# KiloHertzian/Open-Headstage

Hardware: AMD Instinct MI355X
Metric: Msamples/s stereo 48 kHz (4×512-tap HRIR conv + 10-band EQ); % HBM3E peak (higher is better)
Workload: dtype f32

## Files before the change

include/ohs_hip.h:

```cpp
#ifndef OHS_HIP_H
#define OHS_HIP_H

#include <stddef.h>
#include <stdint.h>

#ifdef __cplusplus
extern "C" {
#endif

#define OHS_BLOCK_SIZE 512
#define OHS_FFT_SIZE   1024
#define OHS_MAX_EQ_BANDS 64

enum {
    OHS_OK = 0,
    OHS_ERR_INVALID_ARG = 1,
    OHS_ERR_NO_DEVICE = 2,
    OHS_ERR_HIP = 3,
    OHS_ERR_OUTSIDE_NYQUIST = 4,
    OHS_ERR_NEGATIVE_Q = 5,
    OHS_ERR_ALLOC = 6,
    OHS_ERR_IO = 7,
    OHS_ERR_PARSE = 8,
    OHS_ERR_RCCL = 9
};

enum { OHS_PATH_LSL = 0, OHS_PATH_LSR = 1, OHS_PATH_RSL = 2, OHS_PATH_RSR = 3 };

enum {
    OHS_FILTER_PEAK = 0, OHS_FILTER_LOWSHELF = 1, OHS_FILTER_HIGHSHELF = 2, OHS_FILTER_LOWPASS = 3,
    OHS_FILTER_HIGHPASS = 4, OHS_FILTER_BANDPASS = 5, OHS_FILTER_NOTCH = 6, OHS_FILTER_ALLPASS = 7
};

int         ohs_version(void);
const char *ohs_status_string(int status);
const char *ohs_last_error(void);
int         ohs_device_count(int *count);
int         ohs_device_pci_bus_id(int device, char *out, size_t capacity);

int         ohs_debug_fft1024(int device, const float *in, float *out, int inverse, size_t batch);

typedef struct ohs_engine ohs_engine;

int  ohs_engine_create(int device, ohs_engine **out);
int  ohs_engine_clone(const ohs_engine *src, ohs_engine **out);
void ohs_engine_destroy(ohs_engine *e);
int  ohs_engine_set_ir(ohs_engine *e, int path, const float *ir, size_t len);
int  ohs_engine_process_block(ohs_engine *e, const float *in_l, const float *in_r,
                              float *out_l, float *out_r, size_t n);
int  ohs_engine_num_partitions(const ohs_engine *e, int path, size_t *out);
int  ohs_engine_set_realtime(ohs_engine *e, int enable);
int  ohs_rt_configure(int max_resident_per_device, uint64_t idle_polls);
int  ohs_engine_latency_samples(const ohs_engine *e, size_t n, size_t *latency);
int  ohs_engine_debug_rt_stamps(const ohs_engine *e, uint64_t out[16]);
int  ohs_engine_silent_frames(const ohs_engine *e, uint64_t *frames);
int  ohs_engine_set_flush_denormals(ohs_engine *e, int mode);

typedef struct ohs_eq ohs_eq;

int  ohs_biquad_coeffs(int filter_type, float fs, float fc, float q, float gain_db, float out[5]);
int  ohs_eq_create(int device, size_t num_bands, float fs, ohs_eq **out);
void ohs_eq_destroy(ohs_eq *eq);
int  ohs_eq_update_band(ohs_eq *eq, size_t band, float fs, int filter_type, float fc, float q,
                        float gain_db, int enabled);
int  ohs_eq_set_band_coeffs(ohs_eq *eq, size_t band, const float coeffs[5], int enabled);
int  ohs_eq_get_band_coeffs(const ohs_eq *eq, size_t band, float coeffs[5], int *enabled);
int  ohs_eq_process_block(ohs_eq *eq, float *left, float *right, size_t n);
int  ohs_eq_set_exact_specials(ohs_eq *eq, int enable);
int  ohs_eq_set_flush_denormals(ohs_eq *eq, int mode);
int  ohs_eq_reset(ohs_eq *eq);
int  ohs_eq_frequency_response(const ohs_eq *eq, float fs, const float *freqs, size_t n, float *out);

typedef struct ohs_biquad ohs_biquad;
int  ohs_biquad_create(int device, float initial_sample_rate, ohs_biquad **out);
int  ohs_biquad_clone(const ohs_biquad *src, ohs_biquad **out);
void ohs_biquad_destroy(ohs_biquad *f);
int  ohs_biquad_reset_state(ohs_biquad *f);
int  ohs_biquad_set_enabled(ohs_biquad *f, int enabled);
int  ohs_biquad_update_coeffs(ohs_biquad *f, int filter_type, float sample_rate, float center_freq, float q, float gain_db);
int  ohs_biquad_set_coeffs(ohs_biquad *f, const float coeffs[5]);
int  ohs_biquad_process(ohs_biquad *f, float *samples, size_t n);

typedef struct ohs_band_setting {
    int   enabled;
    int   filter_type;
    float frequency;
    float q;
    float gain;
} ohs_band_setting;
int  ohs_autoeq_parse_csv(const char *path, ohs_band_setting *out, size_t capacity, size_t *count);
int  ohs_autoeq_parse_csv_text(const char *text, size_t len, ohs_band_setting *out, size_t capacity,
                               size_t *count);

typedef struct ohs_sofa ohs_sofa;
int  ohs_sofa_open(const char *path, ohs_sofa **out);
enum { OHS_SOFA_RESAMPLE = 1, OHS_SOFA_LOUDNESS = 2, OHS_SOFA_INTERPOLATE = 4, OHS_SOFA_MYSOFA_DEFAULTS = 7 };
int  ohs_sofa_open_ex(const char *path, unsigned flags, float target_fs, ohs_sofa **out);
int  ohs_sofa_loudness_factor(const ohs_sofa *s, float *factor);
int  ohs_sofa_neighbors(const ohs_sofa *s, size_t m, int out[6]);
void ohs_sofa_close(ohs_sofa *s);
int  ohs_sofa_info(const ohs_sofa *s, size_t *M, size_t *R, size_t *N, float *fs);
int  ohs_sofa_position(const ohs_sofa *s, size_t m, float az_el_r[3]);
int  ohs_sofa_spherical_to_cartesian(const float az_el_r[3], float xyz[3]);
int  ohs_sofa_cartesian_to_spherical(const float xyz[3], float az_el_r[3]);
int  ohs_sofa_nearest(const ohs_sofa *s, float az_deg, float el_deg, float radius_m, size_t *index);
int  ohs_sofa_get_ir(const ohs_sofa *s, size_t m, size_t receiver, float *out, size_t capacity);
int  ohs_sofa_get_hrtf_irs(const ohs_sofa *s, float az_deg, float el_deg, float radius_m, float *left,
                           float *right, size_t capacity, float *delay_left, float *delay_right);
int  ohs_sofa_resample_ir(const float *in, size_t n, float fs_in, float fs_out, float *out, size_t capacity,
                          size_t *out_len);

int  ohs_sofa_speaker_irs(const ohs_sofa *sofa, float az_l, float el_l, float az_r, float el_r, float radius_m, float fs,
                          float *const out[4], size_t capacity, size_t lens[4]);
int  ohs_engine_set_speakers(ohs_engine *e, const ohs_sofa *sofa, float az_l, float el_l, float az_r, float el_r,
                             float radius_m, float fs, unsigned *changed_mask);

int  ohs_chain_process(ohs_engine *e, ohs_eq *eq, int bypass, int eq_enable, float gain,
                       float *left, float *right, size_t n);

typedef struct ohs_batch ohs_batch;

int  ohs_batch_create(int device, size_t n_streams, size_t num_bands, ohs_batch **out);
void ohs_batch_destroy(ohs_batch *b);
int  ohs_batch_set_ir(ohs_batch *b, int path, const float *ir, size_t len);
int  ohs_batch_set_speakers(ohs_batch *b, const ohs_sofa *sofa, float az_l, float el_l, float az_r, float el_r,
                            float radius_m, float fs, unsigned *changed_mask);
int  ohs_batch_set_eq_band_coeffs(ohs_batch *b, size_t band, const float coeffs[5], int enabled);
int  ohs_batch_update_eq_band(ohs_batch *b, size_t band, float fs, int filter_type, float fc,
                              float q, float gain_db, int enabled);
int  ohs_batch_set_stream_eq_band_coeffs(ohs_batch *b, size_t stream, size_t band, const float coeffs[5], int enabled);
int  ohs_batch_update_stream_eq_band(ohs_batch *b, size_t stream, size_t band, float fs, int filter_type, float fc,
                                     float q, float gain_db, int enabled);
int  ohs_batch_share_eq_table(ohs_batch *b);
int  ohs_batch_set_eq_enabled(ohs_batch *b, int eq_enable);
int  ohs_batch_set_eq_exact_specials(ohs_batch *b, int enable);
int  ohs_batch_set_flush_denormals(ohs_batch *b, int mode);
int  ohs_batch_set_gain(ohs_batch *b, float gain);
int  ohs_batch_set_conv_plan(ohs_batch *b, int plan);
enum ohs_conv_kernel {
    OHS_CONV_KERNEL_NONE = 0,
    OHS_CONV_KERNEL_BLOCK512_P1 = 1,
    OHS_CONV_KERNEL_HOP1536_P1 = 2,
    OHS_CONV_KERNEL_BLOCK512_TP = 3,
    OHS_CONV_KERNEL_BLOCK2048 = 4,
    OHS_CONV_KERNEL_SEQUENTIAL = 5,
    OHS_CONV_KERNEL_BLOCK8192 = 6,
    OHS_CONV_KERNEL_COUNT = 8
};
int  ohs_batch_last_conv_plan(const ohs_batch *b, int *kernel, int *ranges_per_stream);
int  ohs_batch_conv_plan_counts(ohs_batch *b, uint64_t counts[8] , int reset);
int  ohs_batch_reset(ohs_batch *b);
int  ohs_batch_process(ohs_batch *b, const float *d_in, float *d_out, size_t n_blocks,
                       size_t stream_stride, size_t channel_stride, void *hip_stream);
int  ohs_batch_set_schedule_tables(ohs_batch *b, size_t n_tables, const float *coeffs, const uint8_t *enabled);
int  ohs_batch_process_scheduled(ohs_batch *b, const float *d_in, float *d_out, size_t n_blocks, size_t stream_stride,
                                 size_t channel_stride, size_t seg_blocks, const unsigned *table_idx, const float *gain,
                                 void *hip_stream);
int  ohs_batch_process_scheduled_streams(ohs_batch *b, const float *d_in, float *d_out, size_t n_blocks, size_t stream_stride,
                                         size_t channel_stride, size_t seg_blocks, const unsigned *table_idx, size_t idx_stride,
                                         const float *gain, size_t gain_stride, void *hip_stream);
enum {
    OHS_EQ_FORM_NONE = 0,
    OHS_EQ_FORM_ROW_RING = 1,
    OHS_EQ_FORM_WAVE_RING = 2,
    OHS_EQ_FORM_CONVEYOR = 3
};
int  ohs_batch_last_eq_form(const ohs_batch *b, int *form, int *scheduled);
int  ohs_batch_process_deferred(ohs_batch *b, const float *d_in, float *d_out, size_t n_blocks,
                                size_t stream_stride, size_t channel_stride, void *hip_stream);
int  ohs_batch_join(ohs_batch *b, void *hip_stream);
int  ohs_batch_process_host(ohs_batch *b, const float *h_in, float *h_out, size_t n_blocks,
                            size_t stream_stride, size_t channel_stride, size_t chunk_blocks);
int  ohs_batch_sync(ohs_batch *b, void *hip_stream);
int  ohs_batch_set_profiling(ohs_batch *b, int enable);
int  ohs_batch_profile_read(ohs_batch *b, double *eq_ms, double *conv_ms, uint64_t *n_calls,
                            uint64_t *eq_launches, uint64_t *conv_launches);
int  ohs_batch_profile_eq_clock(ohs_batch *b, double *shader_ghz, double *wave_us);
int  ohs_batch_algorithmic_bytes(const ohs_batch *b, size_t n_blocks, uint64_t *bytes);
int  ohs_batch_kernel_bytes(const ohs_batch *b, size_t n_blocks, uint64_t *eq_bytes, uint64_t *conv_bytes);

typedef struct ohs_node_batch ohs_node_batch;
int  ohs_node_batch_create(int n_devices, const int *devices, size_t streams_total, size_t num_bands,
                           ohs_node_batch **out);
void ohs_node_batch_destroy(ohs_node_batch *nb);
int  ohs_node_batch_shard(const ohs_node_batch *nb, int slot, int *device, size_t *first_stream, size_t *n_streams);
int  ohs_node_batch_device_batch(ohs_node_batch *nb, int slot, ohs_batch **out);
int  ohs_node_batch_set_tables(ohs_node_batch *nb, const float *const irs[4], const size_t lens[4],
                               const float *eq_coeffs, const int *eq_enabled);
int  ohs_node_batch_set_ir(ohs_node_batch *nb, int path, const float *ir, size_t len);
int  ohs_node_batch_set_speakers(ohs_node_batch *nb, const ohs_sofa *sofa, float az_l, float el_l, float az_r, float el_r,
                                 float radius_m, float fs, unsigned *changed_mask);
int  ohs_node_batch_set_eq_band_coeffs(ohs_node_batch *nb, size_t band, const float coeffs[5], int enabled);
int  ohs_node_batch_set_stream_eq_band_coeffs(ohs_node_batch *nb, size_t stream, size_t band, const float coeffs[5],
                                              int enabled);
int  ohs_node_batch_share_eq_table(ohs_node_batch *nb);
int  ohs_node_batch_set_eq_enabled(ohs_node_batch *nb, int eq_enable);
int  ohs_node_batch_set_gain(ohs_node_batch *nb, float gain);
int  ohs_node_batch_set_conv_plan(ohs_node_batch *nb, int plan);
int  ohs_node_batch_reset(ohs_node_batch *nb);
int  ohs_node_batch_process_host(ohs_node_batch *nb, const float *h_in, float *h_out, size_t n_blocks,
                                 size_t stream_stride, size_t channel_stride, size_t chunk_blocks);
int  ohs_node_batch_process(ohs_node_batch *nb, const float *const d_in[], float *const d_out[], size_t n_blocks,
                            size_t stream_stride, size_t channel_stride);
int  ohs_node_batch_sync(ohs_node_batch *nb);
int  ohs_node_batch_stream(ohs_node_batch *nb, int slot, void **hip_stream);
int  ohs_node_batch_timer_begin(ohs_node_batch *nb);
int  ohs_node_batch_timer_end(ohs_node_batch *nb, float *ms_per_slot);
int  ohs_node_batch_rccl_info(const ohs_node_batch *nb, int *comm_size, int *rccl_loaded);

#ifdef __cplusplus
}
#endif
#endif
```

open_headstage_amd/_ffi.py:

```python
from __future__ import annotations

import ctypes as C
import os

HERE = os.path.dirname(os.path.abspath(__file__))
EXP_LIB_PATH = os.path.join(HERE, "libohs_hip_exp.so")
_env_lib = os.environ.get("OHS_LIB")
LIB_PATH = EXP_LIB_PATH if _env_lib == "exp" else (_env_lib or os.path.join(HERE, "libohs_hip.so"))

OHS_OK = 0
OHS_ERR_INVALID_ARG = 1
OHS_ERR_NO_DEVICE = 2
OHS_ERR_HIP = 3
OHS_ERR_OUTSIDE_NYQUIST = 4
OHS_ERR_NEGATIVE_Q = 5
OHS_ERR_ALLOC = 6
OHS_ERR_IO = 7
OHS_ERR_PARSE = 8
OHS_ERR_RCCL = 9

class BandSettingC(C.Structure):
    _fields_ = [("enabled", C.c_int), ("filter_type", C.c_int), ("frequency", C.c_float),
                ("q", C.c_float), ("gain", C.c_float)]


fp = C.POINTER(C.c_float)
vp = C.c_void_p
vpp = C.POINTER(C.c_void_p)

PROTOTYPES = {
    "ohs_version": (C.c_int, []),
    "ohs_status_string": (C.c_char_p, [C.c_int]),
    "ohs_last_error": (C.c_char_p, []),
    "ohs_device_count": (C.c_int, [C.POINTER(C.c_int)]),
    "ohs_device_pci_bus_id": (C.c_int, [C.c_int, C.c_char_p, C.c_size_t]),
    "ohs_debug_fft1024": (C.c_int, [C.c_int, fp, fp, C.c_int, C.c_size_t]),
    "ohs_engine_create": (C.c_int, [C.c_int, vpp]),
    "ohs_engine_clone": (C.c_int, [vp, vpp]),
    "ohs_engine_destroy": (None, [vp]),
    "ohs_engine_set_ir": (C.c_int, [vp, C.c_int, fp, C.c_size_t]),
    "ohs_engine_process_block": (C.c_int, [vp, vp, vp, vp, vp, C.c_size_t]),
    "ohs_engine_num_partitions": (C.c_int, [vp, C.c_int, C.POINTER(C.c_size_t)]),
    "ohs_engine_set_realtime": (C.c_int, [vp, C.c_int]),
    "ohs_rt_configure": (C.c_int, [C.c_int, C.c_uint64]),
    "ohs_engine_latency_samples": (C.c_int, [vp, C.c_size_t, C.POINTER(C.c_size_t)]),
    "ohs_engine_silent_frames": (C.c_int, [vp, C.POINTER(C.c_uint64)]),
    "ohs_engine_debug_rt_stamps": (C.c_int, [vp, C.POINTER(C.c_uint64)]),
    "ohs_biquad_coeffs": (C.c_int, [C.c_int, C.c_float, C.c_float, C.c_float, C.c_float, fp]),
    "ohs_biquad_create": (C.c_int, [C.c_int, C.c_float, vpp]),
    "ohs_biquad_clone": (C.c_int, [vp, vpp]),
    "ohs_biquad_destroy": (None, [vp]),
    "ohs_biquad_reset_state": (C.c_int, [vp]),
    "ohs_biquad_set_enabled": (C.c_int, [vp, C.c_int]),
    "ohs_biquad_update_coeffs": (C.c_int, [vp, C.c_int, C.c_float, C.c_float, C.c_float, C.c_float]),
    "ohs_biquad_set_coeffs": (C.c_int, [vp, fp]),
    "ohs_biquad_process": (C.c_int, [vp, vp, C.c_size_t]),
    "ohs_eq_create": (C.c_int, [C.c_int, C.c_size_t, C.c_float, vpp]),
    "ohs_eq_destroy": (None, [vp]),
    "ohs_eq_update_band": (C.c_int, [vp, C.c_size_t, C.c_float, C.c_int, C.c_float, C.c_float,
                                     C.c_float, C.c_int]),
    "ohs_eq_set_band_coeffs": (C.c_int, [vp, C.c_size_t, fp, C.c_int]),
    "ohs_eq_get_band_coeffs": (C.c_int, [vp, C.c_size_t, fp, C.POINTER(C.c_int)]),
    "ohs_eq_process_block": (C.c_int, [vp, vp, vp, C.c_size_t]),
    "ohs_eq_reset": (C.c_int, [vp]),
    "ohs_eq_set_exact_specials": (C.c_int, [vp, C.c_int]),
    "ohs_eq_set_flush_denormals": (C.c_int, [vp, C.c_int]),
    "ohs_engine_set_flush_denormals": (C.c_int, [vp, C.c_int]),
    "ohs_batch_set_flush_denormals": (C.c_int, [vp, C.c_int]),
    "ohs_batch_set_eq_exact_specials": (C.c_int, [vp, C.c_int]),
    "ohs_eq_frequency_response": (C.c_int, [vp, C.c_float, fp, C.c_size_t, fp]),
    "ohs_autoeq_parse_csv": (C.c_int, [C.c_char_p, C.POINTER(BandSettingC), C.c_size_t,
                                       C.POINTER(C.c_size_t)]),
    "ohs_autoeq_parse_csv_text": (C.c_int, [C.c_char_p, C.c_size_t, C.POINTER(BandSettingC), C.c_size_t,
                                            C.POINTER(C.c_size_t)]),
    "ohs_sofa_open": (C.c_int, [C.c_char_p, vpp]),
    "ohs_sofa_open_ex": (C.c_int, [C.c_char_p, C.c_uint, C.c_float, vpp]),
    "ohs_sofa_loudness_factor": (C.c_int, [vp, fp]),
    "ohs_sofa_neighbors": (C.c_int, [vp, C.c_size_t, C.POINTER(C.c_int)]),
    "ohs_sofa_close": (None, [vp]),
    "ohs_sofa_info": (C.c_int, [vp, C.POINTER(C.c_size_t), C.POINTER(C.c_size_t), C.POINTER(C.c_size_t),
                                C.POINTER(C.c_float)]),
    "ohs_sofa_position": (C.c_int, [vp, C.c_size_t, fp]),
    "ohs_sofa_spherical_to_cartesian": (C.c_int, [fp, fp]),
    "ohs_sofa_cartesian_to_spherical": (C.c_int, [fp, fp]),
    "ohs_sofa_nearest": (C.c_int, [vp, C.c_float, C.c_float, C.c_float, C.POINTER(C.c_size_t)]),
    "ohs_sofa_get_ir": (C.c_int, [vp, C.c_size_t, C.c_size_t, fp, C.c_size_t]),
    "ohs_sofa_get_hrtf_irs": (C.c_int, [vp, C.c_float, C.c_float, C.c_float, fp, fp, C.c_size_t, fp, fp]),
    "ohs_sofa_resample_ir": (C.c_int, [fp, C.c_size_t, C.c_float, C.c_float, fp, C.c_size_t,
                                       C.POINTER(C.c_size_t)]),
    "ohs_sofa_speaker_irs": (C.c_int, [vp, C.c_float, C.c_float, C.c_float, C.c_float, C.c_float, C.c_float,
                                       C.POINTER(fp), C.c_size_t, C.POINTER(C.c_size_t)]),
    "ohs_engine_set_speakers": (C.c_int, [vp, vp, C.c_float, C.c_float, C.c_float, C.c_float, C.c_float, C.c_float, C.POINTER(C.c_uint)]),
    "ohs_batch_set_speakers": (C.c_int, [vp, vp, C.c_float, C.c_float, C.c_float, C.c_float, C.c_float, C.c_float, C.POINTER(C.c_uint)]),
    "ohs_node_batch_set_speakers": (C.c_int, [vp, vp, C.c_float, C.c_float, C.c_float, C.c_float, C.c_float, C.c_float, C.POINTER(C.c_uint)]),
    "ohs_chain_process": (C.c_int, [vp, vp, C.c_int, C.c_int, C.c_float, vp, vp, C.c_size_t]),
    "ohs_batch_create": (C.c_int, [C.c_int, C.c_size_t, C.c_size_t, vpp]),
    "ohs_batch_destroy": (None, [vp]),
    "ohs_batch_set_ir": (C.c_int, [vp, C.c_int, fp, C.c_size_t]),
    "ohs_batch_set_eq_band_coeffs": (C.c_int, [vp, C.c_size_t, fp, C.c_int]),
    "ohs_batch_update_eq_band": (C.c_int, [vp, C.c_size_t, C.c_float, C.c_int, C.c_float, C.c_float,
                                           C.c_float, C.c_int]),
    "ohs_batch_set_stream_eq_band_coeffs": (C.c_int, [vp, C.c_size_t, C.c_size_t, fp, C.c_int]),
    "ohs_batch_update_stream_eq_band": (C.c_int, [vp, C.c_size_t, C.c_size_t, C.c_float, C.c_int, C.c_float, C.c_float,
                                                  C.c_float, C.c_int]),
    "ohs_batch_share_eq_table": (C.c_int, [vp]),
    "ohs_node_batch_set_stream_eq_band_coeffs": (C.c_int, [vp, C.c_size_t, C.c_size_t, fp, C.c_int]),
    "ohs_node_batch_share_eq_table": (C.c_int, [vp]),
    "ohs_batch_set_eq_enabled": (C.c_int, [vp, C.c_int]),
    "ohs_batch_set_gain": (C.c_int, [vp, C.c_float]),
    "ohs_batch_set_conv_plan": (C.c_int, [vp, C.c_int]),
    "ohs_batch_last_conv_plan": (C.c_int, [vp, C.POINTER(C.c_int), C.POINTER(C.c_int)]),
    "ohs_batch_conv_plan_counts": (C.c_int, [vp, C.POINTER(C.c_uint64), C.c_int]),
    "ohs_batch_profile_eq_clock": (C.c_int, [vp, C.POINTER(C.c_double), C.POINTER(C.c_double)]),
    "ohs_node_batch_set_conv_plan": (C.c_int, [vp, C.c_int]),
    "ohs_batch_reset": (C.c_int, [vp]),
    "ohs_batch_process": (C.c_int, [vp, vp, vp, C.c_size_t, C.c_size_t, C.c_size_t, vp]),
    "ohs_batch_process_deferred": (C.c_int, [vp, vp, vp, C.c_size_t, C.c_size_t, C.c_size_t, vp]),
    "ohs_batch_set_schedule_tables": (C.c_int, [vp, C.c_size_t, fp, C.POINTER(C.c_uint8)]),
    "ohs_batch_process_scheduled": (C.c_int, [vp, vp, vp, C.c_size_t, C.c_size_t, C.c_size_t, C.c_size_t,
                                              C.POINTER(C.c_uint32), fp, vp]),
    "ohs_batch_process_scheduled_streams": (C.c_int, [vp, vp, vp, C.c_size_t, C.c_size_t, C.c_size_t, C.c_size_t,
                                                    C.POINTER(C.c_uint32), C.c_size_t, fp, C.c_size_t, vp]),
    "ohs_batch_last_eq_form": (C.c_int, [vp, C.POINTER(C.c_int), C.POINTER(C.c_int)]),
    "ohs_batch_join": (C.c_int, [vp, vp]),
    "ohs_batch_sync": (C.c_int, [vp, vp]),
    "ohs_batch_process_host": (C.c_int, [vp, vp, vp, C.c_size_t, C.c_size_t, C.c_size_t, C.c_size_t]),
    "ohs_batch_set_profiling": (C.c_int, [vp, C.c_int]),
    "ohs_batch_profile_read": (C.c_int, [vp, C.POINTER(C.c_double), C.POINTER(C.c_double),
                                         C.POINTER(C.c_uint64), C.POINTER(C.c_uint64),
                                         C.POINTER(C.c_uint64)]),
    "ohs_batch_algorithmic_bytes": (C.c_int, [vp, C.c_size_t, C.POINTER(C.c_uint64)]),
    "ohs_batch_kernel_bytes": (C.c_int, [vp, C.c_size_t, C.POINTER(C.c_uint64), C.POINTER(C.c_uint64)]),
    "ohs_node_batch_create": (C.c_int, [C.c_int, C.POINTER(C.c_int), C.c_size_t, C.c_size_t, vpp]),
    "ohs_node_batch_destroy": (None, [vp]),
    "ohs_node_batch_shard": (C.c_int, [vp, C.c_int, C.POINTER(C.c_int), C.POINTER(C.c_size_t), C.POINTER(C.c_size_t)]),
    "ohs_node_batch_device_batch": (C.c_int, [vp, C.c_int, vpp]),
    "ohs_node_batch_set_tables": (C.c_int, [vp, C.POINTER(fp), C.POINTER(C.c_size_t), fp, C.POINTER(C.c_int)]),
    "ohs_node_batch_set_ir": (C.c_int, [vp, C.c_int, fp, C.c_size_t]),
    "ohs_node_batch_set_eq_band_coeffs": (C.c_int, [vp, C.c_size_t, fp, C.c_int]),
    "ohs_node_batch_set_eq_enabled": (C.c_int, [vp, C.c_int]),
    "ohs_node_batch_set_gain": (C.c_int, [vp, C.c_float]),
    "ohs_node_batch_reset": (C.c_int, [vp]),
    "ohs_node_batch_process_host": (C.c_int, [vp, vp, vp, C.c_size_t, C.c_size_t, C.c_size_t, C.c_size_t]),
    "ohs_node_batch_process": (C.c_int, [vp, C.POINTER(C.c_void_p), C.POINTER(C.c_void_p), C.c_size_t, C.c_size_t,
                                         C.c_size_t]),
    "ohs_node_batch_sync": (C.c_int, [vp]),
    "ohs_node_batch_stream": (C.c_int, [vp, C.c_int, vpp]),
    "ohs_node_batch_timer_begin": (C.c_int, [vp]),
    "ohs_node_batch_timer_end": (C.c_int, [vp, fp]),
    "ohs_node_batch_rccl_info": (C.c_int, [vp, C.POINTER(C.c_int), C.POINTER(C.c_int)]),
}


class OhsError(RuntimeError):
    def __init__(self, status: int, detail: str):
        self.status = status
        super().__init__(f"{lib().ohs_status_string(status).decode()} ({status}): {detail}")


DEBUG_PROTOTYPES = {
    "ohs_debug_set_tuning": (C.c_int, [C.c_char_p, C.c_char_p]),
    "ohs_debug_inject_batch_failure": (C.c_int, [C.c_int]),
}

_lib = None
_exp = None


def _load(path: str, extra=None) -> C.CDLL:
    if not os.path.exists(path):
        raise ImportError(
            f"{path} not found: build it with `python -m open_headstage_amd.build` "
            "(hipcc, gfx950). There is no CPU fallback.")
    try:
        import torch
    except ImportError:
        pass
    L = C.CDLL(path)
    for name, (res, args) in {**PROTOTYPES, **(extra or {})}.items():
        fn = getattr(L, name)
        fn.restype = res
        fn.argtypes = args
    return L


def lib() -> C.CDLL:
    global _lib
    if _lib is None:
        _lib = _load(LIB_PATH)
    return _lib


def experiments_lib() -> C.CDLL:
    global _exp
    if _exp is None:
        _exp = _load(EXP_LIB_PATH, DEBUG_PROTOTYPES)
    return _exp


def set_tuning(key: str, value) -> None:
    L = experiments_lib()
    rc = L.ohs_debug_set_tuning(key.encode(), str(value).encode())
    if rc != OHS_OK:
        raise OhsError(rc, L.ohs_last_error().decode(errors="replace"))


def check(status: int, library=None) -> None:
    if status != OHS_OK:
        raise OhsError(status, (library or lib()).ohs_last_error().decode(errors="replace"))
```

open_headstage_amd/csrc/api_batch.hip:

```cpp
#include "api_internal.h"

using namespace ohs;
using namespace ohs_api;
using ohs_host::rbj;

extern "C" {

int ohs_batch_create(int device, size_t n_streams, size_t num_bands, ohs_batch **out)
{
    if (!out) return fail(OHS_ERR_INVALID_ARG, "out is NULL");
    *out = nullptr;
    if (n_streams == 0 || n_streams > (1u << 20)) return fail(OHS_ERR_INVALID_ARG, "n_streams out of range");
    DeviceCtx *ctx = nullptr;
    int rc = get_ctx(device, &ctx);
    if (rc) return rc;
    HIP_TRY(hipSetDevice(device));
    ohs_batch *b = new (std::nothrow) ohs_batch();
    if (!b) return fail(OHS_ERR_ALLOC, "out of host memory");
    b->device = device; b->ctx = ctx;
    if (hipStreamCreateWithFlags(&b->st, hipStreamNonBlocking) != hipSuccess) {
        delete b;
        return fail(OHS_ERR_HIP, "hipStreamCreate failed");
    }
    {
// ... 164 lines not shown
int ohs_batch_conv_plan_counts(ohs_batch *b, uint64_t counts[OHS_CONV_KERNEL_COUNT], int reset)
{
    if (!b || !counts) return fail(OHS_ERR_INVALID_ARG, "NULL argument");
    for (int k = 0; k < OHS_CONV_KERNEL_COUNT; ++k) counts[k] = b->conv.kernel_calls[k];
    if (reset)
        for (int k = 0; k < OHS_CONV_KERNEL_COUNT; ++k) b->conv.kernel_calls[k] = 0;
    return OHS_OK;
}

int ohs_batch_set_gain(ohs_batch *b, float gain)
{
    if (!b) return fail(OHS_ERR_INVALID_ARG, "batch is NULL");
    b->gain = gain;
    return OHS_OK;
}

int ohs_batch_reset(ohs_batch *b)
{
    if (!b) return fail(OHS_ERR_INVALID_ARG, "batch is NULL");
    HIP_TRY(hipSetDevice(b->device));
    DeviceWideSection dws;
    HIP_TRY(hipDeviceSynchronize());
    ConvState &c = b->conv;
    HIP_TRY(hipMemsetAsync(c.d_hist, 0, c.S * (size_t)c.cap * NF * sizeof(float2), b->st));
    HIP_TRY(hipMemsetAsync(c.d_tails, 0, c.S * 2 * 8 * 64 * sizeof(float2), b->st));
    c.tails_lazy = false;
    c.lb_lazy = false; c.lb_valid = 0;
    c.pt_active = false;
    if (c.d_xhist) {
        HIP_TRY(hipMemsetAsync(c.d_xhist, 0, c.S * 2 * (size_t)(2 * c.xh_len) * sizeof(float), b->st));
        c.xh_valid = c.xh_len;
        c.xh_head = 0;
    }
    c.cnt = 0;
    for (int p = 0; p < 4; ++p) c.since[p] = 0;
    int rc = eq_reset(b->eq, b->st);
    if (rc) return rc;
    HIP_TRY(hipStreamSynchronize(b->st));
    b->failed = false;
    b->fail_msg.clear();
    return OHS_OK;
}

static int batch_process_body(ohs_batch *b, const float *d_in, float *d_out, size_t n_blocks,
                              size_t stream_stride, size_t channel_stride, void *hip_stream, bool deferred,
                              const BatchSchedule *sc);

static int batch_process_impl(ohs_batch *b, const float *d_in, float *d_out, size_t n_blocks,
                              size_t stream_stride, size_t channel_stride, void *hip_stream, bool deferred,
                              const BatchSchedule *sc = nullptr)
{
    if (!b || !d_in || !d_out) return fail(OHS_ERR_INVALID_ARG, "NULL argument");
    if (b->failed)
        return fail(OHS_ERR_HIP, "this batch failed in the middle of an earlier call (" + b->fail_msg +
                                     "): its per-stream state is half-advanced; ohs_batch_reset starts it afresh");
    const size_t spans_before = b->spans.size();
    const int rc = batch_process_body(b, d_in, d_out, n_blocks, stream_stride, channel_stride, hip_stream, deferred, sc);
    if (rc == OHS_OK || rc == OHS_ERR_INVALID_ARG) return rc;
    const std::string why = g_err;
    hipStream_t st = (hipStream_t)hip_stream;
    hipEvent_t ev = nullptr;
    if (hipEventCreate(&ev) == hipSuccess) {
        if (hipEventRecord(ev, b->st2) != hipSuccess || hipStreamWaitEvent(st, ev, 0) != hipSuccess)
            hipStreamSynchronize(b->st2);
        b->ev_inflight.push_back(ev);
    } else {
        hipStreamSynchronize(b->st2);
    }
    b->join_pending = false;
    while (b->spans.size() > spans_before) {
        ohs_batch::Span sp = b->spans.back();
        b->spans.pop_back();
        if (sp.a) hipEventDestroy(sp.a);
        if (sp.b) hipEventDestroy(sp.b);
    }
    b->failed = true;
    b->fail_msg = why;
    return fail(rc, why);
}

static int batch_process_body(ohs_batch *b, const float *d_in, float *d_out, size_t n_blocks,
                              size_t stream_stride, size_t channel_stride, void *hip_stream, bool deferred,
                              const BatchSchedule *sc)
{
    if (n_blocks == 0) return OHS_OK;
    if (n_blocks > (size_t)1 << 24) return fail(OHS_ERR_INVALID_ARG, "n_blocks too large");
    const size_t frames = n_blocks * BS;
    if (channel_stride < frames || (b->conv.S > 1 && stream_stride < 2 * frames && stream_stride < channel_stride + frames))
        return fail(OHS_ERR_INVALID_ARG, "strides smaller than the processed region");
    HIP_TRY(hipSetDevice(b->device));
    hipStream_t st = (hipStream_t)hip_stream;
    auto get_event = [&](hipEvent_t *e) -> int {
        if (!b->ev_pool.empty()) { *e = b->ev_pool.back(); b->ev_pool.pop_back(); return OHS_OK; }
        HIP_TRY(hipEventCreate(e));
        return OHS_OK;
    };
    for (size_t i = 0; i < b->ev_inflight.size();) {
        if (hipEventQuery(b->ev_inflight[i]) == hipSuccess) {
            b->ev_pool.push_back(b->ev_inflight[i]);
            b->ev_inflight[i] = b->ev_inflight.back();
            b->ev_inflight.pop_back();
        } else ++i;
    }
    auto span_begin = [&](hipStream_t s_, int kind) -> int {
        if (!b->profiling) return OHS_OK;
        ohs_batch::Span sp; sp.kind = kind; sp.a = nullptr; sp.b = nullptr;
        int rc = get_event(&sp.a); if (rc) return rc;
        rc = get_event(&sp.b); if (rc) return rc;
        HIP_TRY(hipEventRecord(sp.a, s_));
        b->spans.push_back(sp);
        return OHS_OK;
    };
    auto span_end = [&](hipStream_t s_) -> int {
        if (!b->profiling) return OHS_OK;
        HIP_TRY(hipEventRecord(b->spans.back().b, s_));
        return OHS_OK;
    };
    if (b->profiling) b->prof_calls++;

    const bool sched_tabs = sc != nullptr && sc->tab != nullptr;
    bool eq_active = b->eq_enable && eq_any_enabled(b->eq);
    if (sched_tabs) {
        eq_active = false;
        const size_t rows = sc->tab_stride ? b->conv.S : 1;
        for (size_t r = 0; r < rows && b->eq_enable && !eq_active; ++r)
            for (size_t k = 0; k < sc->n_segs && !eq_active; ++k)
                eq_active = eq_schedule_table_any_enabled(b->eq, sc->tab[r * sc->tab_stride + k]);
    }
    ConvGains cg;
    if (sc && sc->d_gain) { cg.tab = sc->d_gain; cg.seg_blocks = (int)sc->seg_blocks; cg.stream_stride = (int)sc->gain_stride; }

    const long long ss = (long long)stream_stride, cs = (long long)channel_stride;
    int rc;
    const bool will_overlap = eq_active && b->overlap && n_blocks >= 64;
    bool chunk_waits = false;
    if (b->join_pending) {
        chunk_waits = will_overlap && b->pend_out == d_out && b->pend_blocks == n_blocks &&
                      b->pend_ss == stream_stride && b->pend_cs == channel_stride;
        if (!chunk_waits) {
            HIP_TRY(hipStreamWaitEvent(st, b->chunk_done[(size_t)b->chunk_done_n - 1], 0));
            b->join_pending = false;
        }
    }
    if (!eq_active) {
#ifdef OHS_EXPERIMENTS
        if (g_inject_batch_failure.load() > 0 && g_inject_batch_failure.fetch_sub(1) == 1)
            return fail(OHS_ERR_HIP, "injected failure (ohs_debug_inject_batch_failure)");
#endif
        rc = span_begin(st, 1); if (rc) return rc;
        rc = conv_launch(b->conv, b->ctx, d_in, ss, cs, d_out, ss, cs, (int)n_blocks, b->gain, st, true, nullptr, nullptr, &cg);
        if (rc) return rc;
        return span_end(st);
    }
    const std::vector<double> &kCut = tuning().overlap_cuts;
    const int nch = (b->overlap && n_blocks >= 64) ? (int)kCut.size() - 1 : 1;
    struct XcdScope {
        ohs_batch *b;
        XcdScope(ohs_batch *b_, int x) : b(b_)
        {
            if (x > 0 && x < 8) { b->eq.xcd_lo = 0; b->eq.xcd_n = x; b->conv.xcd_lo = x; b->conv.xcd_n = 8 - x; }
        }
        ~XcdScope() { b->eq.xcd_lo = 0; b->eq.xcd_n = 8; b->conv.xcd_lo = 0; b->conv.xcd_n = 8; }
    } xcd_scope(b, nch > 1 ? b->xcd_split : 0);
    bool joined = false;
    for (int i = 0; i < nch; ++i) {
        const size_t blk0 = nch == 1 ? 0 : (size_t)(kCut[i] * (double)n_blocks);
        const size_t blk1 = nch == 1 ? n_blocks : (i == nch - 1 ? n_blocks : (size_t)(kCut[i + 1] * (double)n_blocks));
        const size_t off = blk0 * BS;
        const int nb_i = (int)(blk1 - blk0);
        if (nb_i <= 0) {
            if (nch > 1 && deferred) {
                while (b->chunk_done.size() <= (size_t)i) {
                    hipEvent_t ev;
                    HIP_TRY(hipEventCreateWithFlags(&ev, hipEventDisableTiming));
                    b->chunk_done.push_back(ev);
                }
                HIP_TRY(hipEventRecord(b->chunk_done[(size_t)i], b->st2));
            }
            continue;
        }
        if (chunk_waits) HIP_TRY(hipStreamWaitEvent(st, b->chunk_done[(size_t)i], 0));
#ifdef OHS_EXPERIMENTS
        if (g_inject_batch_failure.load() > 0 && g_inject_batch_failure.fetch_sub(1) == 1)
            return fail(OHS_ERR_HIP, "injected failure (ohs_debug_inject_batch_failure)");
#endif
        hipEvent_t ev_a = nullptr, ev_b = nullptr;
        if (b->profiling) {
            ohs_batch::Span sp; sp.kind = 0; sp.a = nullptr; sp.b = nullptr;
            rc = get_event(&sp.a); if (rc) return rc;
            rc = get_event(&sp.b); if (rc) return rc;
            b->spans.push_back(sp);
            ev_a = sp.a; ev_b = sp.b;
        } else if (nch > 1) {
            rc = get_event(&ev_b); if (rc) return rc;
            b->ev_inflight.push_back(ev_b);
        }
        if (sched_tabs && sc->streams)
            rc = eq_launch_scheduled_streams(b->eq, *sc, blk0, (size_t)nb_i, d_in + off, d_out + off, ss, cs, st, ev_a, ev_b);
        else if (sched_tabs) rc = eq_launch_scheduled(b->eq, *sc, blk0, (size_t)nb_i, d_in + off, d_out + off, ss, cs, st, ev_a, ev_b);
        else rc = eq_launch(b->eq, d_in + off, d_out + off, ss, cs, (long long)nb_i * BS, st, nullptr, ev_a, ev_b);
        if (rc) return rc;
        hipStream_t cst = st;
        const bool tail_on_caller = nch > 1 && !deferred && i == nch - 1;
        if (tail_on_caller) {
            hipEvent_t ev;
            rc = get_event(&ev); if (rc) return rc;
            HIP_TRY(hipEventRecord(ev, b->st2));
            HIP_TRY(hipStreamWaitEvent(st, ev, 0));
            b->ev_inflight.push_back(ev);
            joined = true;
        } else if (nch > 1) {
            HIP_TRY(hipStreamWaitEvent(b->st2, ev_b, 0));
            cst = b->st2;
        }
        {
            hipEvent_t cv_a = nullptr, cv_b = nullptr;
            if (b->profiling) {
                ohs_batch::Span sp; sp.kind = 1; sp.a = nullptr; sp.b = nullptr;
                rc = get_event(&sp.a); if (rc) return rc;
                rc = get_event(&sp.b); if (rc) return rc;
                b->spans.push_back(sp);
                cv_a = sp.a; cv_b = sp.b;
            }
            cg.blk_off = (int)blk0;
            rc = conv_launch(b->conv, b->ctx, d_out + off, ss, cs, d_out + off, ss, cs, nb_i, b->gain, cst, true, cv_a, cv_b, &cg);
            if (rc) return rc;
        }
        if (nch > 1 && deferred) {
            while (b->chunk_done.size() <= (size_t)i) {
                hipEvent_t ev;
                HIP_TRY(hipEventCreateWithFlags(&ev, hipEventDisableTiming));
                b->chunk_done.push_back(ev);
            }
            HIP_TRY(hipEventRecord(b->chunk_done[(size_t)i], b->st2));
        }
    }
    b->join_pending = false;
    if (nch > 1 && deferred) {
        b->join_pending = true;
        b->chunk_done_n = nch;
        b->pend_out = d_out; b->pend_blocks = n_blocks; b->pend_ss = stream_stride; b->pend_cs = channel_stride;
    } else if (nch > 1 && !joined) {
        hipEvent_t ev;
        rc = get_event(&ev); if (rc) return rc;
        HIP_TRY(hipEventRecord(ev, b->st2));
        HIP_TRY(hipStreamWaitEvent(st, ev, 0));
        b->ev_inflight.push_back(ev);
    }
    return OHS_OK;
}

int ohs_batch_process(ohs_batch *b, const float *d_in, float *d_out, size_t n_blocks,
                      size_t stream_stride, size_t channel_stride, void *hip_stream)
{
    return batch_process_impl(b, d_in, d_out, n_blocks, stream_stride, channel_stride, hip_stream, false);
}

int ohs_batch_set_schedule_tables(ohs_batch *b, size_t n_tables, const float *coeffs, const uint8_t *enabled)
{
    if (!b) return fail(OHS_ERR_INVALID_ARG, "batch is NULL");
    if (n_tables > 0 && (!coeffs || !enabled)) return fail(OHS_ERR_INVALID_ARG, "NULL argument");
    if (n_tables > ((size_t)1 << 24)) return fail(OHS_ERR_INVALID_ARG, "n_tables too large");
    HIP_TRY(hipSetDevice(b->device));
    return eq_set_schedule_tables(b->eq, n_tables, coeffs, enabled, b->st);
}

int ohs_batch_last_eq_form(const ohs_batch *b, int *form, int *scheduled)
{
    if (!b || !form || !scheduled) return fail(OHS_ERR_INVALID_ARG, "NULL argument");
    *form = b->eq.last_form;
    *scheduled = b->eq.last_scheduled ? 1 : 0;
    return OHS_OK;
}

int ohs_batch_process_scheduled(ohs_batch *b, const float *d_in, float *d_out, size_t n_blocks, size_t stream_stride,
                                size_t channel_stride, size_t seg_blocks, const unsigned *table_idx, const float *gain,
                                void *hip_stream)
{
    if (!b || !d_in || !d_out) return fail(OHS_ERR_INVALID_ARG, "NULL argument");
    if (seg_blocks == 0) return fail(OHS_ERR_INVALID_ARG, "seg_blocks is 0");
    if (n_blocks > (size_t)1 << 24) return fail(OHS_ERR_INVALID_ARG, "n_blocks too large");
    if (b->eq.per_stream)
        return fail(OHS_ERR_INVALID_ARG, "a scheduled call on a handle with per-stream EQ tables is not supported "
                                         "(ohs_batch_share_eq_table goes back to the one shared table)");
    if (table_idx && b->eq.sched_n == 0)
        return fail(OHS_ERR_INVALID_ARG, "table_idx given, but no tables uploaded (ohs_batch_set_schedule_tables)");
    seg_blocks = std::min(seg_blocks, std::max<size_t>(n_blocks, 1));
    const size_t n_segs = (n_blocks + seg_blocks - 1) / seg_blocks;
    if (table_idx)
        for (size_t k = 0; k < n_segs; ++k)
            if (table_idx[k] >= b->eq.sched_n) return fail(OHS_ERR_INVALID_ARG, "table_idx entry out of range");
    if (b->failed || n_blocks == 0)
        return batch_process_impl(b, d_in, d_out, n_blocks, stream_stride, channel_stride, hip_stream, false);
    {
        const size_t frames = n_blocks * BS;
        if (channel_stride < frames || (b->conv.S > 1 && stream_stride < 2 * frames && stream_stride < channel_stride + frames))
            return fail(OHS_ERR_INVALID_ARG, "strides smaller than the processed region");
    }
    auto adopt_table = [&](unsigned t) {
        for (size_t band = 0; band < b->eq.nb; ++band)
            eq_set_shared_band(b->eq, band, &b->eq.sched_coeffs[((size_t)t * b->eq.nb + band) * 5], b->eq.sched_en[(size_t)t * b->eq.nb + band]);
    };
    bool tabs_vary = false, gains_vary = false;
    for (size_t k = 1; k < n_segs; ++k) {
        tabs_vary = tabs_vary || (table_idx && table_idx[k] != table_idx[0]);
        gains_vary = gains_vary || (gain && std::memcmp(&gain[k], &gain[0], sizeof(float)) != 0);
    }
    if (table_idx && !tabs_vary) { adopt_table(table_idx[0]); table_idx = nullptr; }
    if (gain && !gains_vary) { b->gain = gain[0]; gain = nullptr; }
    if (!table_idx && !gain)
        return batch_process_impl(b, d_in, d_out, n_blocks, stream_stride, channel_stride, hip_stream, false);

    HIP_TRY(hipSetDevice(b->device));
    hipStream_t st = (hipStream_t)hip_stream;
    ohs_batch::SchedSlot &slot = b->sched_slot[b->sched_next];
    b->sched_next = (b->sched_next + 1) % ohs_batch::kSchedSlots;
    if (slot.in_use) HIP_TRY(hipEventSynchronize(slot.done));
    slot.in_use = false;
    if (!slot.done) HIP_TRY(hipEventCreateWithFlags(&slot.done, hipEventDisableTiming));
    if (slot.cap < n_segs) {
        if (slot.h) hipHostFree(slot.h);
        if (slot.d) {
            DeviceWideSection dws;
            hipFree(slot.d);
        }
        slot.h = nullptr; slot.d = nullptr; slot.cap = 0;
        const size_t cap = std::max<size_t>(1024, n_segs + n_segs / 2);
        HIP_TRY(hipHostMalloc(reinterpret_cast<void **>(&slot.h), 2 * cap * sizeof(unsigned), hipHostMallocDefault));
        HIP_TRY(hipMalloc(reinterpret_cast<void **>(&slot.d), 2 * cap * sizeof(unsigned)));
        slot.cap = cap;
    }
    BatchSchedule sc;
    sc.seg_blocks = seg_blocks; sc.n_segs = n_segs; sc.tab = table_idx; sc.gain = gain;
    if (table_idx) {
        std::memcpy(slot.h, table_idx, n_segs * sizeof(unsigned));
        HIP_TRY(hipMemcpyAsync(slot.d, slot.h, n_segs * sizeof(unsigned), hipMemcpyHostToDevice, st));
        sc.d_tab = slot.d;
    }
    if (gain) {
        std::memcpy(slot.h + slot.cap, gain, n_segs * sizeof(float));
        HIP_TRY(hipMemcpyAsync(slot.d + slot.cap, slot.h + slot.cap, n_segs * sizeof(float), hipMemcpyHostToDevice, st));
        sc.d_gain = reinterpret_cast<const float *>(slot.d + slot.cap);
    }
    const int rc = batch_process_impl(b, d_in, d_out, n_blocks, stream_stride, channel_stride, hip_stream, false, &sc);
    if (hipEventRecord(slot.done, st) == hipSuccess) slot.in_use = true;
    else hipStreamSynchronize(st);
    if (rc) return rc;
    if (table_idx) adopt_table(table_idx[n_segs - 1]);
    if (gain) b->gain = gain[n_segs - 1];
    return OHS_OK;
}

int ohs_batch_process_scheduled_streams(ohs_batch *b, const float *d_in, float *d_out, size_t n_blocks, size_t stream_stride,
                                        size_t channel_stride, size_t seg_blocks, const unsigned *table_idx, size_t idx_stride,
                                        const float *gain, size_t gain_stride, void *hip_stream)
{
    if (!b || !d_in || !d_out) return fail(OHS_ERR_INVALID_ARG, "NULL argument");
    if (seg_blocks == 0) return fail(OHS_ERR_INVALID_ARG, "seg_blocks is 0");
    if (n_blocks > (size_t)1 << 24) return fail(OHS_ERR_INVALID_ARG, "n_blocks too large");
    if (table_idx && b->eq.per_stream)
        return fail(OHS_ERR_INVALID_ARG, "table_idx on a handle with static per-stream EQ tables is not supported: the schedule "
                                         "tables take their place (ohs_batch_share_eq_table), or pass table_idx = NULL");
    if (table_idx && b->eq.sched_n == 0)
        return fail(OHS_ERR_INVALID_ARG, "table_idx given, but no tables uploaded (ohs_batch_set_schedule_tables)");
    seg_blocks = std::min(seg_blocks, std::max<size_t>(n_blocks, 1));
    const size_t n_segs = (n_blocks + seg_blocks - 1) / seg_blocks, S = b->conv.S;
    if ((table_idx && idx_stride != 0 && idx_stride < n_segs) || (gain && gain_stride != 0 && gain_stride < n_segs))
        return fail(OHS_ERR_INVALID_ARG, "a row stride is 0 (one row for all streams) or >= the number of segments");
    if (S * n_segs > (size_t)0x7fffffff) return fail(OHS_ERR_INVALID_ARG, "schedule too large");
    if (!table_idx) idx_stride = 0;
    if (!gain) gain_stride = 0;
    BatchSchedule sc;
    sc.seg_blocks = seg_blocks; sc.n_segs = n_segs; sc.streams = true;
    if (table_idx) {
        sc.tab = table_idx; sc.tab_stride = idx_stride;
        if (!eq_schedule_streams_scan(b->eq, sc)) return fail(OHS_ERR_INVALID_ARG, "table_idx entry out of range");
    }
    if (b->failed || n_blocks == 0)
        return batch_process_impl(b, d_in, d_out, n_blocks, stream_stride, channel_stride, hip_stream, false);
    {
        const size_t frames = n_blocks * BS;
        if (channel_stride < frames || (S > 1 && stream_stride < 2 * frames && stream_stride < channel_stride + frames))
            return fail(OHS_ERR_INVALID_ARG, "strides smaller than the processed region");
    }
    auto rows_equal = [&](const void *base, size_t stride) {
        const unsigned *p = static_cast<const unsigned *>(base);
        for (size_t s = 1; s < S; ++s)
            if (std::memcmp(p + s * stride, p, n_segs * sizeof(unsigned)) != 0) return false;
        return true;
    };
    if (idx_stride && rows_equal(table_idx, idx_stride)) idx_stride = 0;
    if (gain_stride && rows_equal(gain, gain_stride)) gain_stride = 0;
    struct Restore {
        ohs_batch *b;
        std::vector<float> coeffs; std::vector<int> en; float gain;
        explicit Restore(ohs_batch *b_) : b(b_), coeffs(b_->eq.coeffs), en(b_->eq.en.begin(), b_->eq.en.end()), gain(b_->gain) {}
        ~Restore()
        {
            b->gain = gain;
            if (!b->eq.per_stream)
                for (size_t band = 0; band < b->eq.nb; ++band) eq_set_shared_band(b->eq, band, &coeffs[5 * band], en[band]);
        }
    } restore(b);
    if (!idx_stride && !gain_stride && !b->eq.per_stream)
        return ohs_batch_process_scheduled(b, d_in, d_out, n_blocks, stream_stride, channel_stride, seg_blocks, table_idx, gain, hip_stream);
    auto adopt_table = [&](unsigned t) {
        for (size_t band = 0; band < b->eq.nb; ++band)
            eq_set_shared_band(b->eq, band, &b->eq.sched_coeffs[((size_t)t * b->eq.nb + band) * 5], b->eq.sched_en[(size_t)t * b->eq.nb + band]);
    };
    if (table_idx && !idx_stride) {
        bool vary = false;
        for (size_t k = 1; k < n_segs; ++k) vary = vary || table_idx[k] != table_idx[0];
        if (!vary) { adopt_table(table_idx[0]); table_idx = nullptr; }
    }
    if (gain && !gain_stride) {
        bool vary = false;
        for (size_t k = 1; k < n_segs; ++k) vary = vary || std::memcmp(&gain[k], &gain[0], sizeof(float)) != 0;
// ... 336 lines not shown
```

open_headstage_amd/csrc/eq_quad_ring_asm.inc:

```
#define EQ_QUAD_RING_K 8
#define EQ_QUAD_RING_LOOP \
    "s_mov_b32 vcc_lo, -1\n" \
    "s_mov_b32 vcc_hi, 0x3333ffff\n" \
    ".p2align 5\n" \
    "1:\n" \
    "v_add_f32_dpp v3, v4, v5 wave_ror:1 row_mask:0xf bank_mask:0xf\n" \
    "v_mul_f32_dpp v4, v2, v8 quad_perm:[0,0,0,3] row_mask:0xf bank_mask:0xf\n" \
    "v_nop_e64\n" \
    "v_mul_f32_dpp v6, v3, v7 quad_perm:[0,0,3,3] row_mask:0xf bank_mask:0xf\n" \
    "v_sub_f32_dpp v5, v3, v6 quad_perm:[0,0,1,2] row_mask:0xf bank_mask:0xf\n" \
    "v_add_f32_dpp v2, v4, v5 wave_ror:1 row_mask:0xf bank_mask:0xf\n" \
    "v_mul_f32_dpp v4, v3, v8 quad_perm:[0,0,0,3] row_mask:0xf bank_mask:0xf\n" \
    "v_nop_e64\n" \
    "v_mul_f32_dpp v6, v2, v7 quad_perm:[0,0,3,3] row_mask:0xf bank_mask:0xf\n" \
    "v_sub_f32_dpp v5, v2, v6 quad_perm:[0,0,1,2] row_mask:0xf bank_mask:0xf\n" \
    "v_add_f32_dpp v3, v4, v5 wave_ror:1 row_mask:0xf bank_mask:0xf\n" \
    "v_mul_f32_dpp v4, v2, v8 quad_perm:[0,0,0,3] row_mask:0xf bank_mask:0xf\n" \
    "v_nop_e64\n" \
    "v_mul_f32_dpp v6, v3, v7 quad_perm:[0,0,3,3] row_mask:0xf bank_mask:0xf\n" \
    "v_sub_f32_dpp v5, v3, v6 quad_perm:[0,0,1,2] row_mask:0xf bank_mask:0xf\n" \
    "v_add_f32_dpp v2, v4, v5 wave_ror:1 row_mask:0xf bank_mask:0xf\n" \
    "v_mul_f32_dpp v4, v3, v8 quad_perm:[0,0,0,3] row_mask:0xf bank_mask:0xf\n" \
    "v_nop_e64\n" \
    "v_mul_f32_dpp v6, v2, v7 quad_perm:[0,0,3,3] row_mask:0xf bank_mask:0xf\n" \
    "v_sub_f32_dpp v5, v2, v6 quad_perm:[0,0,1,2] row_mask:0xf bank_mask:0xf\n" \
    "v_add_f32_dpp v3, v4, v5 wave_ror:1 row_mask:0xf bank_mask:0xf\n" \
    "v_mul_f32_dpp v4, v2, v8 quad_perm:[0,0,0,3] row_mask:0xf bank_mask:0xf\n" \
    "v_nop_e64\n" \
    "v_mul_f32_dpp v6, v3, v7 quad_perm:[0,0,3,3] row_mask:0xf bank_mask:0xf\n" \
    "v_sub_f32_dpp v5, v3, v6 quad_perm:[0,0,1,2] row_mask:0xf bank_mask:0xf\n" \
    "v_add_f32_dpp v2, v4, v5 wave_ror:1 row_mask:0xf bank_mask:0xf\n" \
    "v_mul_f32_dpp v4, v3, v8 quad_perm:[0,0,0,3] row_mask:0xf bank_mask:0xf\n" \
    "v_nop_e64\n" \
    "v_mul_f32_dpp v6, v2, v7 quad_perm:[0,0,3,3] row_mask:0xf bank_mask:0xf\n" \
    "v_sub_f32_dpp v5, v2, v6 quad_perm:[0,0,1,2] row_mask:0xf bank_mask:0xf\n" \
    "v_add_f32_dpp v3, v4, v5 wave_ror:1 row_mask:0xf bank_mask:0xf\n" \
    "v_mul_f32_dpp v4, v2, v8 quad_perm:[0,0,0,3] row_mask:0xf bank_mask:0xf\n" \
    "v_nop_e64\n" \
    "v_mul_f32_dpp v6, v3, v7 quad_perm:[0,0,3,3] row_mask:0xf bank_mask:0xf\n" \
    "v_sub_f32_dpp v5, v3, v6 quad_perm:[0,0,1,2] row_mask:0xf bank_mask:0xf\n" \
    "v_add_f32_dpp v2, v4, v5 wave_ror:1 row_mask:0xf bank_mask:0xf\n" \
    "v_mul_f32_dpp v4, v3, v8 quad_perm:[0,0,0,3] row_mask:0xf bank_mask:0xf\n" \
    "buffer_store_dword v2, v0, %[rout], 0 offen offset:64\n" \
    "v_mul_f32_dpp v6, v2, v7 quad_perm:[0,0,3,3] row_mask:0xf bank_mask:0xf\n" \
    "v_sub_f32_dpp v5, v2, v6 quad_perm:[0,0,1,2] row_mask:0xf bank_mask:0xf\n" \
    "v_add_f32_dpp v3, v4, v5 wave_ror:1 row_mask:0xf bank_mask:0xf\n" \
    "v_mul_f32_dpp v4, v2, v8 quad_perm:[0,0,0,3] row_mask:0xf bank_mask:0xf\n" \
    "v_cndmask_b32_dpp v4, v11, v4, vcc quad_perm:[0,1,0,1] row_mask:0xf bank_mask:0xf\n" \
    "v_mul_f32_dpp v6, v3, v7 quad_perm:[0,0,3,3] row_mask:0xf bank_mask:0xf\n" \
    "v_sub_f32_dpp v5, v3, v6 quad_perm:[0,0,1,2] row_mask:0xf bank_mask:0xf\n" \
    "v_add_f32_dpp v2, v4, v5 wave_ror:1 row_mask:0xf bank_mask:0xf\n" \
    "v_mul_f32_dpp v4, v3, v8 quad_perm:[0,0,0,3] row_mask:0xf bank_mask:0xf\n" \
    "buffer_load_dword v11, v1, %[rin], 0 offen offset:512\n" \
    "v_mul_f32_dpp v6, v2, v7 quad_perm:[0,0,3,3] row_mask:0xf bank_mask:0xf\n" \
    "v_sub_f32_dpp v5, v2, v6 quad_perm:[0,0,1,2] row_mask:0xf bank_mask:0xf\n" \
    "v_add_f32_dpp v3, v4, v5 wave_ror:1 row_mask:0xf bank_mask:0xf\n" \
    "v_mul_f32_dpp v4, v2, v8 quad_perm:[0,0,0,3] row_mask:0xf bank_mask:0xf\n" \
    "v_nop_e64\n" \
    "v_mul_f32_dpp v6, v3, v7 quad_perm:[0,0,3,3] row_mask:0xf bank_mask:0xf\n" \
    "v_sub_f32_dpp v5, v3, v6 quad_perm:[0,0,1,2] row_mask:0xf bank_mask:0xf\n" \
    "v_add_f32_dpp v2, v4, v5 wave_ror:1 row_mask:0xf bank_mask:0xf\n" \
    "v_mul_f32_dpp v4, v3, v8 quad_perm:[0,0,0,3] row_mask:0xf bank_mask:0xf\n" \
    "v_nop_e64\n" \
    "v_mul_f32_dpp v6, v2, v7 quad_perm:[0,0,3,3] row_mask:0xf bank_mask:0xf\n" \
    "v_sub_f32_dpp v5, v2, v6 quad_perm:[0,0,1,2] row_mask:0xf bank_mask:0xf\n" \
    "v_add_f32_dpp v3, v4, v5 wave_ror:1 row_mask:0xf bank_mask:0xf\n" \
    "v_mul_f32_dpp v4, v2, v8 quad_perm:[0,0,0,3] row_mask:0xf bank_mask:0xf\n" \
    "v_nop_e64\n" \
    "v_mul_f32_dpp v6, v3, v7 quad_perm:[0,0,3,3] row_mask:0xf bank_mask:0xf\n" \
    "v_sub_f32_dpp v5, v3, v6 quad_perm:[0,0,1,2] row_mask:0xf bank_mask:0xf\n" \
    "v_add_f32_dpp v2, v4, v5 wave_ror:1 row_mask:0xf bank_mask:0xf\n" \
    "v_mul_f32_dpp v4, v3, v8 quad_perm:[0,0,0,3] row_mask:0xf bank_mask:0xf\n" \
    "s_waitcnt vmcnt(21)\n" \
    "s_nop 0\n" \
    "v_mul_f32_dpp v6, v2, v7 quad_perm:[0,0,3,3] row_mask:0xf bank_mask:0xf\n" \
    "v_sub_f32_dpp v5, v2, v6 quad_perm:[0,0,1,2] row_mask:0xf bank_mask:0xf\n" \
    "v_add_f32_dpp v3, v4, v5 wave_ror:1 row_mask:0xf bank_mask:0xf\n" \
    "v_mul_f32_dpp v4, v2, v8 quad_perm:[0,0,0,3] row_mask:0xf bank_mask:0xf\n" \
    "buffer_store_dword v3, v0, %[rout], 0 offen offset:92\n" \
    "v_mul_f32_dpp v6, v3, v7 quad_perm:[0,0,3,3] row_mask:0xf bank_mask:0xf\n" \
    "v_sub_f32_dpp v5, v3, v6 quad_perm:[0,0,1,2] row_mask:0xf bank_mask:0xf\n" \
    "v_add_f32_dpp v2, v4, v5 wave_ror:1 row_mask:0xf bank_mask:0xf\n" \
    "v_mul_f32_dpp v4, v3, v8 quad_perm:[0,0,0,3] row_mask:0xf bank_mask:0xf\n" \
    "v_cndmask_b32_dpp v4, v12, v4, vcc quad_perm:[0,1,2,3] row_mask:0xf bank_mask:0xf\n" \
    "v_mul_f32_dpp v6, v2, v7 quad_perm:[0,0,3,3] row_mask:0xf bank_mask:0xf\n" \
    "v_sub_f32_dpp v5, v2, v6 quad_perm:[0,0,1,2] row_mask:0xf bank_mask:0xf\n" \
    "v_add_f32_dpp v3, v4, v5 wave_ror:1 row_mask:0xf bank_mask:0xf\n" \
    "v_mul_f32_dpp v4, v2, v8 quad_perm:[0,0,0,3] row_mask:0xf bank_mask:0xf\n" \
    "v_nop_e64\n" \
    "v_mul_f32_dpp v6, v3, v7 quad_perm:[0,0,3,3] row_mask:0xf bank_mask:0xf\n" \
    "v_sub_f32_dpp v5, v3, v6 quad_perm:[0,0,1,2] row_mask:0xf bank_mask:0xf\n" \
    "v_add_f32_dpp v2, v4, v5 wave_ror:1 row_mask:0xf bank_mask:0xf\n" \
    "v_mul_f32_dpp v4, v3, v8 quad_perm:[0,0,0,3] row_mask:0xf bank_mask:0xf\n" \
    "v_nop_e64\n" \
    "v_mul_f32_dpp v6, v2, v7 quad_perm:[0,0,3,3] row_mask:0xf bank_mask:0xf\n" \
    "v_sub_f32_dpp v5, v2, v6 quad_perm:[0,0,1,2] row_mask:0xf bank_mask:0xf\n" \
    "v_add_f32_dpp v3, v4, v5 wave_ror:1 row_mask:0xf bank_mask:0xf\n" \
    "v_mul_f32_dpp v4, v2, v8 quad_perm:[0,0,0,3] row_mask:0xf bank_mask:0xf\n" \
    "v_nop_e64\n" \
    "v_mul_f32_dpp v6, v3, v7 quad_perm:[0,0,3,3] row_mask:0xf bank_mask:0xf\n" \
    "v_sub_f32_dpp v5, v3, v6 quad_perm:[0,0,1,2] row_mask:0xf bank_mask:0xf\n" \
    "v_add_f32_dpp v2, v4, v5 wave_ror:1 row_mask:0xf bank_mask:0xf\n" \
    "v_mul_f32_dpp v4, v3, v8 quad_perm:[0,0,0,3] row_mask:0xf bank_mask:0xf\n" \
    "v_nop_e64\n" \
    "v_mul_f32_dpp v6, v2, v7 quad_perm:[0,0,3,3] row_mask:0xf bank_mask:0xf\n" \
    "v_sub_f32_dpp v5, v2, v6 quad_perm:[0,0,1,2] row_mask:0xf bank_mask:0xf\n" \
    "v_add_f32_dpp v3, v4, v5 wave_ror:1 row_mask:0xf bank_mask:0xf\n" \
    "v_mul_f32_dpp v4, v2, v8 quad_perm:[0,0,0,3] row_mask:0xf bank_mask:0xf\n" \
    "v_nop_e64\n" \
    "v_mul_f32_dpp v6, v3, v7 quad_perm:[0,0,3,3] row_mask:0xf bank_mask:0xf\n" \
    "v_sub_f32_dpp v5, v3, v6 quad_perm:[0,0,1,2] row_mask:0xf bank_mask:0xf\n" \
    "v_add_f32_dpp v2, v4, v5 wave_ror:1 row_mask:0xf bank_mask:0xf\n" \
    "v_mul_f32_dpp v4, v3, v8 quad_perm:[0,0,0,3] row_mask:0xf bank_mask:0xf\n" \
    "v_nop_e64\n" \
    "v_mul_f32_dpp v6, v2, v7 quad_perm:[0,0,3,3] row_mask:0xf bank_mask:0xf\n" \
    "v_sub_f32_dpp v5, v2, v6 quad_perm:[0,0,1,2] row_mask:0xf bank_mask:0xf\n" \
    "v_add_f32_dpp v3, v4, v5 wave_ror:1 row_mask:0xf bank_mask:0xf\n" \
    "v_mul_f32_dpp v4, v2, v8 quad_perm:[0,0,0,3] row_mask:0xf bank_mask:0xf\n" \
    "v_nop_e64\n" \
    "v_mul_f32_dpp v6, v3, v7 quad_perm:[0,0,3,3] row_mask:0xf bank_mask:0xf\n" \
    "v_sub_f32_dpp v5, v3, v6 quad_perm:[0,0,1,2] row_mask:0xf bank_mask:0xf\n" \
    "v_add_f32_dpp v2, v4, v5 wave_ror:1 row_mask:0xf bank_mask:0xf\n" \
    "v_mul_f32_dpp v4, v3, v8 quad_perm:[0,0,0,3] row_mask:0xf bank_mask:0xf\n" \
    "buffer_store_dword v2, v0, %[rout], 0 offen offset:128\n" \
    "v_mul_f32_dpp v6, v2, v7 quad_perm:[0,0,3,3] row_mask:0xf bank_mask:0xf\n" \
    "v_sub_f32_dpp v5, v2, v6 quad_perm:[0,0,1,2] row_mask:0xf bank_mask:0xf\n" \
    "v_add_f32_dpp v3, v4, v5 wave_ror:1 row_mask:0xf bank_mask:0xf\n" \
    "v_mul_f32_dpp v4, v2, v8 quad_perm:[0,0,0,3] row_mask:0xf bank_mask:0xf\n" \
    "v_cndmask_b32_dpp v4, v12, v4, vcc quad_perm:[0,1,0,1] row_mask:0xf bank_mask:0xf\n" \
    "v_mul_f32_dpp v6, v3, v7 quad_perm:[0,0,3,3] row_mask:0xf bank_mask:0xf\n" \
    "v_sub_f32_dpp v5, v3, v6 quad_perm:[0,0,1,2] row_mask:0xf bank_mask:0xf\n" \
    "v_add_f32_dpp v2, v4, v5 wave_ror:1 row_mask:0xf bank_mask:0xf\n" \
    "v_mul_f32_dpp v4, v3, v8 quad_perm:[0,0,0,3] row_mask:0xf bank_mask:0xf\n" \
    "buffer_load_dword v12, v1, %[rin], 0 offen offset:576\n" \
    "v_mul_f32_dpp v6, v2, v7 quad_perm:[0,0,3,3] row_mask:0xf bank_mask:0xf\n" \
    "v_sub_f32_dpp v5, v2, v6 quad_perm:[0,0,1,2] row_mask:0xf bank_mask:0xf\n" \
    "v_add_f32_dpp v3, v4, v5 wave_ror:1 row_mask:0xf bank_mask:0xf\n" \
    "v_mul_f32_dpp v4, v2, v8 quad_perm:[0,0,0,3] row_mask:0xf bank_mask:0xf\n" \
    "v_nop_e64\n" \
    "v_mul_f32_dpp v6, v3, v7 quad_perm:[0,0,3,3] row_mask:0xf bank_mask:0xf\n" \
    "v_sub_f32_dpp v5, v3, v6 quad_perm:[0,0,1,2] row_mask:0xf bank_mask:0xf\n" \
    "v_add_f32_dpp v2, v4, v5 wave_ror:1 row_mask:0xf bank_mask:0xf\n" \
    "v_mul_f32_dpp v4, v3, v8 quad_perm:[0,0,0,3] row_mask:0xf bank_mask:0xf\n" \
    "v_nop_e64\n" \
    "v_mul_f32_dpp v6, v2, v7 quad_perm:[0,0,3,3] row_mask:0xf bank_mask:0xf\n" \
    "v_sub_f32_dpp v5, v2, v6 quad_perm:[0,0,1,2] row_mask:0xf bank_mask:0xf\n" \
    "v_add_f32_dpp v3, v4, v5 wave_ror:1 row_mask:0xf bank_mask:0xf\n" \
    "v_mul_f32_dpp v4, v2, v8 quad_perm:[0,0,0,3] row_mask:0xf bank_mask:0xf\n" \
    "v_nop_e64\n" \
    "v_mul_f32_dpp v6, v3, v7 quad_perm:[0,0,3,3] row_mask:0xf bank_mask:0xf\n" \
    "v_sub_f32_dpp v5, v3, v6 quad_perm:[0,0,1,2] row_mask:0xf bank_mask:0xf\n" \
    "v_add_f32_dpp v2, v4, v5 wave_ror:1 row_mask:0xf bank_mask:0xf\n" \
    "v_mul_f32_dpp v4, v3, v8 quad_perm:[0,0,0,3] row_mask:0xf bank_mask:0xf\n" \
    "s_waitcnt vmcnt(21)\n" \
    "s_nop 0\n" \
    "v_mul_f32_dpp v6, v2, v7 quad_perm:[0,0,3,3] row_mask:0xf bank_mask:0xf\n" \
// ... 345 lines not shown
    "v_add_f32_dpp v3, v4, v5 wave_ror:1 row_mask:0xf bank_mask:0xf\n" \
    "v_mul_f32_dpp v4, v2, v8 quad_perm:[0,0,0,3] row_mask:0xf bank_mask:0xf\n" \
    "v_nop_e64\n" \
    "v_mul_f32_dpp v6, v3, v7 quad_perm:[0,0,3,3] row_mask:0xf bank_mask:0xf\n" \
    "v_sub_f32_dpp v5, v3, v6 quad_perm:[0,0,1,2] row_mask:0xf bank_mask:0xf\n" \
    "v_add_f32_dpp v2, v4, v5 wave_ror:1 row_mask:0xf bank_mask:0xf\n" \
    "v_mul_f32_dpp v4, v3, v8 quad_perm:[0,0,0,3] row_mask:0xf bank_mask:0xf\n" \
    "v_nop_e64\n" \
    "v_mul_f32_dpp v6, v2, v7 quad_perm:[0,0,3,3] row_mask:0xf bank_mask:0xf\n" \
    "v_sub_f32_dpp v5, v2, v6 quad_perm:[0,0,1,2] row_mask:0xf bank_mask:0xf\n" \
    "v_add_f32_dpp v3, v4, v5 wave_ror:1 row_mask:0xf bank_mask:0xf\n" \
    "v_mul_f32_dpp v4, v2, v8 quad_perm:[0,0,0,3] row_mask:0xf bank_mask:0xf\n" \
    "v_nop_e64\n" \
    "v_mul_f32_dpp v6, v3, v7 quad_perm:[0,0,3,3] row_mask:0xf bank_mask:0xf\n" \
    "v_sub_f32_dpp v5, v3, v6 quad_perm:[0,0,1,2] row_mask:0xf bank_mask:0xf\n" \
    "v_add_f32_dpp v2, v4, v5 wave_ror:1 row_mask:0xf bank_mask:0xf\n" \
    "v_mul_f32_dpp v4, v3, v8 quad_perm:[0,0,0,3] row_mask:0xf bank_mask:0xf\n" \
    "v_nop_e64\n" \
    "v_mul_f32_dpp v6, v2, v7 quad_perm:[0,0,3,3] row_mask:0xf bank_mask:0xf\n" \
    "v_sub_f32_dpp v5, v2, v6 quad_perm:[0,0,1,2] row_mask:0xf bank_mask:0xf\n" \
    "v_add_f32_dpp v3, v4, v5 wave_ror:1 row_mask:0xf bank_mask:0xf\n" \
    "v_mul_f32_dpp v4, v2, v8 quad_perm:[0,0,0,3] row_mask:0xf bank_mask:0xf\n" \
    "v_nop_e64\n" \
    "v_mul_f32_dpp v6, v3, v7 quad_perm:[0,0,3,3] row_mask:0xf bank_mask:0xf\n" \
    "v_sub_f32_dpp v5, v3, v6 quad_perm:[0,0,1,2] row_mask:0xf bank_mask:0xf\n" \
    "v_add_f32_dpp v2, v4, v5 wave_ror:1 row_mask:0xf bank_mask:0xf\n" \
    "v_mul_f32_dpp v4, v3, v8 quad_perm:[0,0,0,3] row_mask:0xf bank_mask:0xf\n" \
    "buffer_store_dword v2, v0, %[rout], 0 offen offset:448\n" \
    "v_mul_f32_dpp v6, v2, v7 quad_perm:[0,0,3,3] row_mask:0xf bank_mask:0xf\n" \
    "v_sub_f32_dpp v5, v2, v6 quad_perm:[0,0,1,2] row_mask:0xf bank_mask:0xf\n" \
    "v_add_f32_dpp v3, v4, v5 wave_ror:1 row_mask:0xf bank_mask:0xf\n" \
    "v_mul_f32_dpp v4, v2, v8 quad_perm:[0,0,0,3] row_mask:0xf bank_mask:0xf\n" \
    "v_cndmask_b32_dpp v4, v17, v4, vcc quad_perm:[0,1,0,1] row_mask:0xf bank_mask:0xf\n" \
    "v_mul_f32_dpp v6, v3, v7 quad_perm:[0,0,3,3] row_mask:0xf bank_mask:0xf\n" \
    "v_sub_f32_dpp v5, v3, v6 quad_perm:[0,0,1,2] row_mask:0xf bank_mask:0xf\n" \
    "v_add_f32_dpp v2, v4, v5 wave_ror:1 row_mask:0xf bank_mask:0xf\n" \
    "v_mul_f32_dpp v4, v3, v8 quad_perm:[0,0,0,3] row_mask:0xf bank_mask:0xf\n" \
    "buffer_load_dword v17, v1, %[rin], 0 offen offset:896\n" \
    "v_mul_f32_dpp v6, v2, v7 quad_perm:[0,0,3,3] row_mask:0xf bank_mask:0xf\n" \
    "v_sub_f32_dpp v5, v2, v6 quad_perm:[0,0,1,2] row_mask:0xf bank_mask:0xf\n" \
    "v_add_f32_dpp v3, v4, v5 wave_ror:1 row_mask:0xf bank_mask:0xf\n" \
    "v_mul_f32_dpp v4, v2, v8 quad_perm:[0,0,0,3] row_mask:0xf bank_mask:0xf\n" \
    "v_nop_e64\n" \
    "v_mul_f32_dpp v6, v3, v7 quad_perm:[0,0,3,3] row_mask:0xf bank_mask:0xf\n" \
    "v_sub_f32_dpp v5, v3, v6 quad_perm:[0,0,1,2] row_mask:0xf bank_mask:0xf\n" \
    "v_add_f32_dpp v2, v4, v5 wave_ror:1 row_mask:0xf bank_mask:0xf\n" \
    "v_mul_f32_dpp v4, v3, v8 quad_perm:[0,0,0,3] row_mask:0xf bank_mask:0xf\n" \
    "v_nop_e64\n" \
    "v_mul_f32_dpp v6, v2, v7 quad_perm:[0,0,3,3] row_mask:0xf bank_mask:0xf\n" \
    "v_sub_f32_dpp v5, v2, v6 quad_perm:[0,0,1,2] row_mask:0xf bank_mask:0xf\n" \
    "v_add_f32_dpp v3, v4, v5 wave_ror:1 row_mask:0xf bank_mask:0xf\n" \
    "v_mul_f32_dpp v4, v2, v8 quad_perm:[0,0,0,3] row_mask:0xf bank_mask:0xf\n" \
    "v_nop_e64\n" \
    "v_mul_f32_dpp v6, v3, v7 quad_perm:[0,0,3,3] row_mask:0xf bank_mask:0xf\n" \
    "v_sub_f32_dpp v5, v3, v6 quad_perm:[0,0,1,2] row_mask:0xf bank_mask:0xf\n" \
    "v_add_f32_dpp v2, v4, v5 wave_ror:1 row_mask:0xf bank_mask:0xf\n" \
    "v_mul_f32_dpp v4, v3, v8 quad_perm:[0,0,0,3] row_mask:0xf bank_mask:0xf\n" \
    "s_waitcnt vmcnt(21)\n" \
    "s_nop 0\n" \
    "v_mul_f32_dpp v6, v2, v7 quad_perm:[0,0,3,3] row_mask:0xf bank_mask:0xf\n" \
    "v_sub_f32_dpp v5, v2, v6 quad_perm:[0,0,1,2] row_mask:0xf bank_mask:0xf\n" \
    "v_add_f32_dpp v3, v4, v5 wave_ror:1 row_mask:0xf bank_mask:0xf\n" \
    "v_mul_f32_dpp v4, v2, v8 quad_perm:[0,0,0,3] row_mask:0xf bank_mask:0xf\n" \
    "buffer_store_dword v3, v0, %[rout], 0 offen offset:476\n" \
    "v_mul_f32_dpp v6, v3, v7 quad_perm:[0,0,3,3] row_mask:0xf bank_mask:0xf\n" \
    "v_sub_f32_dpp v5, v3, v6 quad_perm:[0,0,1,2] row_mask:0xf bank_mask:0xf\n" \
    "v_add_f32_dpp v2, v4, v5 wave_ror:1 row_mask:0xf bank_mask:0xf\n" \
    "v_mul_f32_dpp v4, v3, v8 quad_perm:[0,0,0,3] row_mask:0xf bank_mask:0xf\n" \
    "v_cndmask_b32_dpp v4, v18, v4, vcc quad_perm:[0,1,2,3] row_mask:0xf bank_mask:0xf\n" \
    "v_mul_f32_dpp v6, v2, v7 quad_perm:[0,0,3,3] row_mask:0xf bank_mask:0xf\n" \
    "v_sub_f32_dpp v5, v2, v6 quad_perm:[0,0,1,2] row_mask:0xf bank_mask:0xf\n" \
    "v_add_f32_dpp v3, v4, v5 wave_ror:1 row_mask:0xf bank_mask:0xf\n" \
    "v_mul_f32_dpp v4, v2, v8 quad_perm:[0,0,0,3] row_mask:0xf bank_mask:0xf\n" \
    "v_nop_e64\n" \
    "v_mul_f32_dpp v6, v3, v7 quad_perm:[0,0,3,3] row_mask:0xf bank_mask:0xf\n" \
    "v_sub_f32_dpp v5, v3, v6 quad_perm:[0,0,1,2] row_mask:0xf bank_mask:0xf\n" \
    "v_add_f32_dpp v2, v4, v5 wave_ror:1 row_mask:0xf bank_mask:0xf\n" \
    "v_mul_f32_dpp v4, v3, v8 quad_perm:[0,0,0,3] row_mask:0xf bank_mask:0xf\n" \
    "v_nop_e64\n" \
    "v_mul_f32_dpp v6, v2, v7 quad_perm:[0,0,3,3] row_mask:0xf bank_mask:0xf\n" \
    "v_sub_f32_dpp v5, v2, v6 quad_perm:[0,0,1,2] row_mask:0xf bank_mask:0xf\n" \
    "v_add_f32_dpp v3, v4, v5 wave_ror:1 row_mask:0xf bank_mask:0xf\n" \
    "v_mul_f32_dpp v4, v2, v8 quad_perm:[0,0,0,3] row_mask:0xf bank_mask:0xf\n" \
    "v_nop_e64\n" \
    "v_mul_f32_dpp v6, v3, v7 quad_perm:[0,0,3,3] row_mask:0xf bank_mask:0xf\n" \
    "v_sub_f32_dpp v5, v3, v6 quad_perm:[0,0,1,2] row_mask:0xf bank_mask:0xf\n" \
    "v_add_f32_dpp v2, v4, v5 wave_ror:1 row_mask:0xf bank_mask:0xf\n" \
    "v_mul_f32_dpp v4, v3, v8 quad_perm:[0,0,0,3] row_mask:0xf bank_mask:0xf\n" \
    "v_nop_e64\n" \
    "v_mul_f32_dpp v6, v2, v7 quad_perm:[0,0,3,3] row_mask:0xf bank_mask:0xf\n" \
    "v_sub_f32_dpp v5, v2, v6 quad_perm:[0,0,1,2] row_mask:0xf bank_mask:0xf\n" \
    "v_add_f32_dpp v3, v4, v5 wave_ror:1 row_mask:0xf bank_mask:0xf\n" \
    "v_mul_f32_dpp v4, v2, v8 quad_perm:[0,0,0,3] row_mask:0xf bank_mask:0xf\n" \
    "v_nop_e64\n" \
    "v_mul_f32_dpp v6, v3, v7 quad_perm:[0,0,3,3] row_mask:0xf bank_mask:0xf\n" \
    "v_sub_f32_dpp v5, v3, v6 quad_perm:[0,0,1,2] row_mask:0xf bank_mask:0xf\n" \
    "v_add_f32_dpp v2, v4, v5 wave_ror:1 row_mask:0xf bank_mask:0xf\n" \
    "v_mul_f32_dpp v4, v3, v8 quad_perm:[0,0,0,3] row_mask:0xf bank_mask:0xf\n" \
    "v_nop_e64\n" \
    "v_mul_f32_dpp v6, v2, v7 quad_perm:[0,0,3,3] row_mask:0xf bank_mask:0xf\n" \
    "v_sub_f32_dpp v5, v2, v6 quad_perm:[0,0,1,2] row_mask:0xf bank_mask:0xf\n" \
    "v_add_f32_dpp v3, v4, v5 wave_ror:1 row_mask:0xf bank_mask:0xf\n" \
    "v_mul_f32_dpp v4, v2, v8 quad_perm:[0,0,0,3] row_mask:0xf bank_mask:0xf\n" \
    "v_nop_e64\n" \
    "v_mul_f32_dpp v6, v3, v7 quad_perm:[0,0,3,3] row_mask:0xf bank_mask:0xf\n" \
    "v_sub_f32_dpp v5, v3, v6 quad_perm:[0,0,1,2] row_mask:0xf bank_mask:0xf\n" \
    "v_add_f32_dpp v2, v4, v5 wave_ror:1 row_mask:0xf bank_mask:0xf\n" \
    "v_mul_f32_dpp v4, v3, v8 quad_perm:[0,0,0,3] row_mask:0xf bank_mask:0xf\n" \
    "buffer_store_dword v2, v0, %[rout], 0 offen offset:512\n" \
    "v_mul_f32_dpp v6, v2, v7 quad_perm:[0,0,3,3] row_mask:0xf bank_mask:0xf\n" \
    "v_sub_f32_dpp v5, v2, v6 quad_perm:[0,0,1,2] row_mask:0xf bank_mask:0xf\n" \
    "v_add_f32_dpp v3, v4, v5 wave_ror:1 row_mask:0xf bank_mask:0xf\n" \
    "v_mul_f32_dpp v4, v2, v8 quad_perm:[0,0,0,3] row_mask:0xf bank_mask:0xf\n" \
    "v_cndmask_b32_dpp v4, v18, v4, vcc quad_perm:[0,1,0,1] row_mask:0xf bank_mask:0xf\n" \
    "v_mul_f32_dpp v6, v3, v7 quad_perm:[0,0,3,3] row_mask:0xf bank_mask:0xf\n" \
    "v_sub_f32_dpp v5, v3, v6 quad_perm:[0,0,1,2] row_mask:0xf bank_mask:0xf\n" \
    "v_add_f32_dpp v2, v4, v5 wave_ror:1 row_mask:0xf bank_mask:0xf\n" \
    "v_mul_f32_dpp v4, v3, v8 quad_perm:[0,0,0,3] row_mask:0xf bank_mask:0xf\n" \
    "buffer_load_dword v18, v1, %[rin], 0 offen offset:960\n" \
    "v_mul_f32_dpp v6, v2, v7 quad_perm:[0,0,3,3] row_mask:0xf bank_mask:0xf\n" \
    "v_sub_f32_dpp v5, v2, v6 quad_perm:[0,0,1,2] row_mask:0xf bank_mask:0xf\n" \
    "v_add_f32_dpp v3, v4, v5 wave_ror:1 row_mask:0xf bank_mask:0xf\n" \
    "v_mul_f32_dpp v4, v2, v8 quad_perm:[0,0,0,3] row_mask:0xf bank_mask:0xf\n" \
    "v_add_u32_e64 v1, v1, v9\n" \
    "v_mul_f32_dpp v6, v3, v7 quad_perm:[0,0,3,3] row_mask:0xf bank_mask:0xf\n" \
    "v_sub_f32_dpp v5, v3, v6 quad_perm:[0,0,1,2] row_mask:0xf bank_mask:0xf\n" \
    "v_add_f32_dpp v2, v4, v5 wave_ror:1 row_mask:0xf bank_mask:0xf\n" \
    "v_mul_f32_dpp v4, v3, v8 quad_perm:[0,0,0,3] row_mask:0xf bank_mask:0xf\n" \
    "v_add_u32_e64 v0, v0, v10\n" \
    "v_mul_f32_dpp v6, v2, v7 quad_perm:[0,0,3,3] row_mask:0xf bank_mask:0xf\n" \
    "v_sub_f32_dpp v5, v2, v6 quad_perm:[0,0,1,2] row_mask:0xf bank_mask:0xf\n" \
    "v_add_f32_dpp v3, v4, v5 wave_ror:1 row_mask:0xf bank_mask:0xf\n" \
    "v_mul_f32_dpp v4, v2, v8 quad_perm:[0,0,0,3] row_mask:0xf bank_mask:0xf\n" \
    "v_nop_e64\n" \
    "v_mul_f32_dpp v6, v3, v7 quad_perm:[0,0,3,3] row_mask:0xf bank_mask:0xf\n" \
    "v_sub_f32_dpp v5, v3, v6 quad_perm:[0,0,1,2] row_mask:0xf bank_mask:0xf\n" \
    "v_add_f32_dpp v2, v4, v5 wave_ror:1 row_mask:0xf bank_mask:0xf\n" \
    "v_mul_f32_dpp v4, v3, v8 quad_perm:[0,0,0,3] row_mask:0xf bank_mask:0xf\n" \
    "s_waitcnt vmcnt(21)\n" \
    "s_add_u32 %[cnt], %[cnt], 1\n" \
    "v_mul_f32_dpp v6, v2, v7 quad_perm:[0,0,3,3] row_mask:0xf bank_mask:0xf\n" \
    "v_sub_f32_dpp v5, v2, v6 quad_perm:[0,0,1,2] row_mask:0xf bank_mask:0xf\n" \
    "v_add_f32_dpp v3, v4, v5 wave_ror:1 row_mask:0xf bank_mask:0xf\n" \
    "v_mul_f32_dpp v4, v2, v8 quad_perm:[0,0,0,3] row_mask:0xf bank_mask:0xf\n" \
    "buffer_store_dword v3, v0, %[rout], 0 offen offset:28\n" \
    "v_mul_f32_dpp v6, v3, v7 quad_perm:[0,0,3,3] row_mask:0xf bank_mask:0xf\n" \
    "v_sub_f32_dpp v5, v3, v6 quad_perm:[0,0,1,2] row_mask:0xf bank_mask:0xf\n" \
    "v_add_f32_dpp v2, v4, v5 wave_ror:1 row_mask:0xf bank_mask:0xf\n" \
    "v_mul_f32_dpp v4, v3, v8 quad_perm:[0,0,0,3] row_mask:0xf bank_mask:0xf\n" \
    "v_cndmask_b32_dpp v4, v11, v4, vcc quad_perm:[0,1,2,3] row_mask:0xf bank_mask:0xf\n" \
    "v_mul_f32_dpp v6, v2, v7 quad_perm:[0,0,3,3] row_mask:0xf bank_mask:0xf\n" \
    "v_sub_f32_dpp v5, v2, v6 quad_perm:[0,0,1,2] row_mask:0xf bank_mask:0xf\n" \
    "s_cbranch_scc0 1b\n" \
    "s_waitcnt vmcnt(0)\n" \
    "s_nop 1\n"
```

open_headstage_amd/csrc/eq_quad_ring_body.hpp:

```cpp
#pragma once
#include "kernels.h"
#include "eq_ring64_body.hpp"
#include "eq_quad_ring_asm.inc"

namespace ohs {

constexpr int kQuadGroup = 16;
constexpr int kQuadK = EQ_QUAD_RING_K;
constexpr int kQp0003 = 0xC0, kQp0033 = 0xF0, kQp0012 = 0x90, kQp0101 = 0x44;

struct QuadRegs { float Z0, Z1, Zp, G, P; };

__device__ __forceinline__ void eq_quad_ring_wave(const float *in, float *out, long long stream_stride, long long ch_stride,
                                                  long long n, int n_chains, int nb, const EqPassTable &tab,
                                                  float *__restrict__ state, long long chain)
{
    constexpr int G = kQuadGroup, K = kQuadK;
    static_assert(K == 8, "the operand list below names x0 .. x7");
    if (chain >= n_chains) return;
    const int lane = threadIdx.x & 63, q = lane >> 2, role = lane & 3;
    const int n32 = (int)n;
    const bool band = q < nb, conv = q >= 12;
    const int j = band ? q : 0;
    const float C1 = role < 2 ? 1.0f : !band ? 0.0f : role == 2 ? tab.a2[j] : tab.a1[j];
    const float C2 = !band ? (role < 2 ? 0.0f : 1.0f) : role == 0 ? tab.b2[j] : role == 1 ? tab.b1[j] : role == 2 ? tab.b0[j] : 1.0f;
    const long long base = (chain >> 1) * stream_stride + (chain & 1) * ch_stride;
    const float *src0 = in + base;
    float *dst0 = out + base;
    float *state0 = state + chain * (kEqStateSlots * 2);
    const bool st_band = band && role >= 2;
    const unsigned state_off = (unsigned)(tab.slot[j] * 2 + (role == 2 ? 1 : 0)) * 4u;
    const float s_init = st_band ? ring2_ld(state0, state_off) : 0.0f;
    float s_save = s_init;
    const int t_in = 4 * q + 2;
    const int xs = (role == 0 ? 71 : role == 1 ? 69 : role == 2 ? 62 : 60) - 4 * q;
    const int ss = (role == 0 ? -1 : -3) - 4 * q;
    const bool st_lane = conv && (role == 0 || role == 3), inj_lane = conv && role >= 2;
    auto load_x = [&](int g) -> float {
        const int i = g * G + xs;
        return (conv && (unsigned)i < (unsigned)n32) ? ring2_ld(src0, (unsigned)i * 4u) : 0.0f;
    };
    QuadRegs r = {0.0f, 0.0f, 0.0f, 0.0f, 0.0f};
    float xcur = load_x(-1), xnext = load_x(0);

    const int g_hi = (n32 + 1) / G;
    const int iters = g_hi - 5 >= K ? (g_hi - 5) / K : 0;
    const int g1 = iters ? g_hi : -1, g0 = iters ? g_hi - iters * K : -1;
    float x2 = 0.0f, x3 = 0.0f, x4 = 0.0f, x5 = 0.0f, x6 = 0.0f, x7 = 0.0f;
    if (iters) {
        x2 = load_x(g0 + 2); x3 = load_x(g0 + 3); x4 = load_x(g0 + 4);
        x5 = load_x(g0 + 5); x6 = load_x(g0 + 6); x7 = load_x(g0 + 7);
    }

    auto group_cpp = [&](int g) {
        const float xnext2 = load_x(g + 2);
        auto step = [&](float &zc, const float zo, int s) {
            const int stp = g * G + s;
            zc = dpp_mov<kWaveRor1>(r.Zp, r.Zp) + r.G;
            r.Zp = dpp_mov<kQp0003>(zo, zo) * C2;
            if (s == 8 || s == 15) {
                const int yi = stp + ss;
                if (st_lane && (unsigned)yi < (unsigned)n32) ring2_st(dst0, (unsigned)yi * 4u, zc);
            } else if (s == 9) {
                const float xb = dpp_mov<kQp0101>(xcur, xcur);
                r.Zp = inj_lane ? xb : r.Zp;
            } else if (s == 16) {
                r.Zp = inj_lane ? xnext : r.Zp;
            }
            r.P = dpp_mov<kQp0033>(zc, zc) * C1;
            r.G = dpp_mov<kQp0012>(zc, zc) - r.P;
            if (st_band && stp == t_in) r.G = s_init;
            if (st_band && stp == n32 + t_in) s_save = r.G;
        };
#pragma unroll 1
        for (int s = 1; s <= G; s += 2) {
            step(r.Z1, r.Z0, s);
            step(r.Z0, r.Z1, s + 1);
        }
        xcur = xnext;
        xnext = xnext2;
    };

    const int g_total = (n32 + 62 + G - 1) / G;
    int g = -1;
    const int head_end = iters ? g0 : g_total;
#pragma unroll 1
    for (; g < head_end; ++g) group_cpp(g);
    if (iters) {
        const unsigned bytes = (unsigned)n32 * 4u;
        const ring64_rsrc_t rin = ring64_rsrc(src0, bytes), rout = ring64_rsrc(dst0, bytes);
        unsigned voff_st = st_lane ? (unsigned)(G * (g0 - 1) + 8 + ss) * 4u : 0xFFFFF000u;
        unsigned voff_ld = conv ? (unsigned)(G * g0 + xs) * 4u : 0xFFFFF000u;
        const unsigned inc_ld = conv ? 4u * G * K : 0u, inc_st = st_lane ? 4u * G * K : 0u;
        unsigned cnt = 0u - (unsigned)__builtin_amdgcn_readfirstlane(iters);
        asm volatile(
            "s_nop 4\n"
            EQ_QUAD_RING_LOOP
            : [Z0] "+{v2}"(r.Z0), [Z1] "+{v3}"(r.Z1), [Zp] "+{v4}"(r.Zp), [Gr] "+{v5}"(r.G), [P] "+{v6}"(r.P),
              [vs] "+{v0}"(voff_st), [vl] "+{v1}"(voff_ld), [x0] "+{v11}"(xcur), [x1] "+{v12}"(xnext), [x2] "+{v13}"(x2),
              [x3] "+{v14}"(x3), [x4] "+{v15}"(x4), [x5] "+{v16}"(x5), [x6] "+{v17}"(x6), [x7] "+{v18}"(x7), [cnt] "+s"(cnt)
            : [C1] "{v7}"(C1), [C2] "{v8}"(C2), [incl] "{v9}"(inc_ld), [incs] "{v10}"(inc_st), [rin] "s"(rin), [rout] "s"(rout)
            : "memory", "scc", "vcc");
        g = g1;
#pragma unroll 1
        for (; g < g_total; ++g) group_cpp(g);
    }
    if (st_band) ring2_st(state0, state_off, s_save);
}

}
```

open_headstage_amd/csrc/tuning.cpp:

```cpp
#include "tuning.h"

#include <algorithm>
#include <cstdio>
#include <cstdlib>
#include <mutex>

namespace ohs {

namespace {
Tuning g_tuning;

#ifdef OHS_EXPERIMENTS
bool parse_ints(const std::string &v, int *out, int n)
{
    const char *p = v.c_str();
    for (int i = 0; i < n; ++i) {
        char *end = nullptr;
        const long x = strtol(p, &end, 10);
        if (end == p) return false;
        out[i] = (int)x;
        p = (*end == ',') ? end + 1 : end;
    }
    return true;
}

const struct { const char *env, *key; } kEnvKeys[] = {
    {"OHS_P1_TARGET_WAVES", "p1_target_waves"}, {"OHS_P1_ROUNDS", "p1_rounds"}, {"OHS_P1_OWN_TAILS", "p1_own_tails"},
    {"OHS_P1_STAGGER", "p1_stagger"}, {"OHS_P1_PRIO", "p1_prio"}, {"OHS_P1_WEIGHTS", "p1_weights"},
    {"OHS_P1_LAZY_STATE", "p1_lazy_state"}, {"OHS_P1_XCD", "p1_xcd"}, {"OHS_EQ_XCD", "eq_xcd"},
    {"OHS_EQ_CONVEYOR", "eq_conveyor"}, {"OHS_EQ_RING_V1", "eq_ring_v1"}, {"OHS_EQ_NO_PRIO", "eq_no_prio"}, {"OHS_EQ_FORM", "eq_form"},
    {"OHS_EQ_WG_WAVES", "eq_wg_waves"}, {"OHS_EQ_LDS", "eq_lds"}, {"OHS_NO_OVERLAP", "no_overlap"},
    {"OHS_FORCE_OVERLAP", "force_overlap"}, {"OHS_XCD_SPLIT", "xcd_split"}, {"OHS_OVERLAP_CUTS", "overlap_cuts"},
    {"OHS_CONV_CU_MASK", "conv_cu_mask"}, {"OHS_MAC_NO_XCD", "mac_no_xcd"}, {"OHS_HOST_PIPE_TRACE", "host_pipe_trace"},
    {"OHS_HOST_PIPE_FLAT_PRIORITIES", "host_pipe_flat_priorities"}, {"OHS_RT_MAX_RESIDENT", "rt_max_resident"},
    {"OHS_RT_IDLE_POLLS", "rt_idle_polls"}, {"OHS_RT_POLL_SLEEP", "rt_poll_sleep"},
    {"OHS_NODE_SHARED_DEVICE", "node_shared_device_rehearsal"},
};
std::once_flag g_env_once;
void load_env()
{
    for (const auto &e : kEnvKeys)
        if (const char *v = getenv(e.env))
            if (!tuning_set(e.key, v)) fprintf(stderr, "[ohs experiments] %s=%s ignored\n", e.env, v);
}
#endif
}

const Tuning &tuning()
{
#ifdef OHS_EXPERIMENTS
    std::call_once(g_env_once, load_env);
#endif
    return g_tuning;
}

Tuning &tuning_rt()
{
#ifdef OHS_EXPERIMENTS
    std::call_once(g_env_once, load_env);
#endif
    return g_tuning;
}

#ifdef OHS_EXPERIMENTS
bool tuning_set(const std::string &key, const std::string &value)
{
    Tuning &t = g_tuning;
    int v[4] = {0, 0, 0, 0};
    auto one = [&](int *dst) { if (!parse_ints(value, v, 1)) return false; *dst = v[0]; return true; };
    if (key == "p1_target_waves") { t.p1_target_waves = atoll(value.c_str()); return true; }
    if (key == "p1_rounds") return one(&t.p1_rounds) && (t.p1_rounds = (t.p1_rounds >= 1 && t.p1_rounds <= 4) ? t.p1_rounds : 1);
    if (key == "p1_own_tails") return one(&t.p1_own_tails);
    if (key == "p1_stagger") return one(&t.p1_stagger);
    if (key == "p1_prio") return one(&t.p1_prio);
    if (key == "p1_lazy_state") return one(&t.p1_lazy_state);
    if (key == "p1_weights") {
        if (!parse_ints(value, v, 4)) return false;
        for (int i = 0; i < 4; ++i) if (v[i] <= 0 || v[i] >= 100000) return false;
        for (int i = 0; i < 4; ++i) t.p1_weights[i] = v[i];
        return true;
    }
    if (key == "p1_xcd" || key == "eq_xcd") {
        int *lo = key == "p1_xcd" ? &t.p1_xcd_lo : &t.eq_xcd_lo, *n = key == "p1_xcd" ? &t.p1_xcd_n : &t.eq_xcd_n;
        if (value.empty() || value == "off") { *lo = 0; *n = 0; return true; }
        if (!parse_ints(value, v, 2) || v[1] < 1 || v[0] < 0 || v[0] + v[1] > 8) return false;
        *lo = v[0]; *n = v[1];
        return true;
    }
    if (key == "eq_conveyor") return one(&t.eq_conveyor);
    if (key == "eq_ring_v1") return one(&t.eq_ring_v1);
    if (key == "eq_no_prio") return one(&t.eq_no_prio);
    if (key == "eq_form") return one(&t.eq_form);
    if (key == "eq_wg_waves") {
        if (!one(&t.eq_wg_waves)) return false;
        const int w = t.eq_wg_waves;
        if (!(w == 0 || w == 1 || w == 2 || w == 4 || w == 8 || w == 16)) { t.eq_wg_waves = 0; return false; }
        return true;
    }
    if (key == "eq_lds") { if (!one(&t.eq_lds)) return false; if (t.eq_lds < 0 || t.eq_lds > 65536) t.eq_lds = 0; return true; }
    if (key == "no_overlap") return one(&t.no_overlap);
    if (key == "force_overlap") return one(&t.force_overlap);
    if (key == "xcd_split") { if (!one(&t.xcd_split)) return false; if (t.xcd_split < 0 || t.xcd_split > 7) t.xcd_split = 0; return true; }
    if (key == "overlap_cuts") {
        std::vector<double> c = {0.0};
        const char *p = value.c_str();
        while (*p && c.size() < 16) {
            char *end = nullptr;
            const double x = strtod(p, &end);
            if (end == p) break;
            if (x > c.back() && x < 1.0) c.push_back(x);
            p = (*end == ',') ? end + 1 : end;
        }
        c.push_back(1.0);
        if (c.size() < 3) return false;
        t.overlap_cuts = c;
        return true;
    }
    if (key == "conv_cu_mask") {
        std::vector<unsigned> m;
        const char *p = value.c_str();
        while (*p) {
            char *end = nullptr;
            const unsigned long x = strtoul(p, &end, 16);
            if (end == p) break;
            m.push_back((unsigned)x);
            p = (*end == ',') ? end + 1 : end;
        }
        t.conv_cu_mask = m;
        return true;
    }
    if (key == "mac_no_xcd") return one(&t.mac_no_xcd);
    if (key == "lb_skip") return one(&t.lb_skip);
    if (key == "xb_min_p") return one(&t.xb_min_p);
    if (key == "xb_min_blocks") return one(&t.xb_min_blocks);
    if (key == "xb_min_streams_p2") return one(&t.xb_min_streams_p2);
    if (key == "xb_stagger") { if (!one(&t.xb_stagger)) return false; t.xb_stagger = std::max(0, std::min(t.xb_stagger, 64)); return true; }
    if (key == "xb_run") return one(&t.xb_run);
    if (key == "xb_skip") return one(&t.xb_skip);
    if (key == "lb_seg_windows") { if (!one(&t.lb_seg_windows)) return false; if (t.lb_seg_windows < 64) t.lb_seg_windows = 64; return true; }
    if (key == "lb_min_p") { if (!one(&t.lb_min_p)) return false; if (t.lb_min_p < 2) t.lb_min_p = 2; return true; }
    if (key == "host_pipe_trace") return one(&t.host_pipe_trace);
    if (key == "host_pipe_flat_priorities") return one(&t.host_pipe_flat_priorities);
    if (key == "node_shared_device_rehearsal") return one(&t.node_shared_device_rehearsal);
    if (key == "node_inject_table_failure_slot") return one(&t.node_inject_table_failure_slot);
    if (key == "rt_max_resident") { int v = 0; if (!one(&v)) return false; rt_max_resident_store(v); return true; }
    if (key == "rt_idle_polls") { rt_idle_polls_store(strtoull(value.c_str(), nullptr, 10)); return true; }
    if (key == "rt_poll_sleep") { if (!one(v)) return false; t.rt_poll_sleep = (unsigned)v[0]; return true; }
    return false;
}
#endif

}
```

open_headstage_amd/csrc/tuning.h:

```cpp
#pragma once
#include "experiments.h"

#include <string>
#include <vector>

namespace ohs {

struct Tuning {
    long long p1_target_waves = 0;
    int p1_rounds = 1;
    int p1_own_tails = 1;
    int p1_stagger = 0;
    int p1_prio = 0;
    int p1_weights[4] = {1425, 1128, 825, 622};
    int p1_lazy_state = 1;
    int p1_xcd_lo = 0, p1_xcd_n = 0;
    int eq_xcd_lo = 0, eq_xcd_n = 0;
    int eq_conveyor = 0;
    int eq_ring_v1 = 0;
    int eq_no_prio = 0;
    int eq_form = 0;
    int eq_wg_waves = 0;
    int eq_lds = 0;
    int no_overlap = 0, force_overlap = 0;
    int xcd_split = 0;
    std::vector<double> overlap_cuts = {0.0, 0.25, 0.5, 0.75, 0.92, 0.98, 1.0};
    std::vector<unsigned> conv_cu_mask;
    int mac_no_xcd = 0;
    int lb_min_p = 2;
    int lb_seg_windows = 131072;
    int xb_min_p = 2;
    int xb_min_blocks = 128;
    int xb_min_streams_p2 = 32;
    int xb_stagger = 1;
    int xb_skip = 0;
    int xb_run = 0;
    int lb_skip = 0;
    int host_pipe_trace = 0, host_pipe_flat_priorities = 0;
    int node_shared_device_rehearsal = 0;
    int node_inject_table_failure_slot = 0;
    int rt_max_resident = -1;
    unsigned long long rt_idle_polls = 3000000ull;
    unsigned rt_poll_sleep = 0;
};

const Tuning &tuning();
Tuning &tuning_rt();
inline int rt_max_resident_load() { return __atomic_load_n(&tuning().rt_max_resident, __ATOMIC_RELAXED); }
inline unsigned long long rt_idle_polls_load() { return __atomic_load_n(&tuning().rt_idle_polls, __ATOMIC_RELAXED); }
inline void rt_max_resident_store(int v) { __atomic_store_n(&tuning_rt().rt_max_resident, v, __ATOMIC_RELAXED); }
inline void rt_idle_polls_store(unsigned long long v) { __atomic_store_n(&tuning_rt().rt_idle_polls, v, __ATOMIC_RELAXED); }
#ifdef OHS_EXPERIMENTS
bool tuning_set(const std::string &key, const std::string &value);
#endif

}
```

Baseline: 26130.

## Geometric overlap chunk plan for wave-ring EQ and asm remainder tail

Replaces the fixed fractional overlap cut table with a planner that, when the EQ pass uses the wave-ring form, sizes chunks geometrically from a small tail chunk, with a minimum block floor. The aim is to shorten the final non-overlapped EQ/convolution stage and pipeline the two stages better. The hand-written DPP ring assembly also gains a remainder path, so leftover groups that are not a multiple of the unroll factor stay in asm instead of falling back to the C++ loop. A test-only plan query API is exported. Costs are more code complexity, the risk of chunk sizes that suit some block counts poorly, and correctness risk in the register rotation of the asm tail.

After: 26130 (median of 2 runs). About the same (+0.0%).

```diff
diff --git a/include/ohs_hip.h b/include/ohs_hip.h
--- a/include/ohs_hip.h
+++ b/include/ohs_hip.h
@@ -166,6 +166,7 @@
     OHS_EQ_FORM_CONVEYOR = 3
 };
 int  ohs_batch_last_eq_form(const ohs_batch *b, int *form, int *scheduled);
+int  ohs_batch_overlap_plan(size_t n_blocks, int wave_ring, size_t *cuts, size_t cap, size_t *n_chunks);
 int  ohs_batch_process_deferred(ohs_batch *b, const float *d_in, float *d_out, size_t n_blocks,
                                 size_t stream_stride, size_t channel_stride, void *hip_stream);
 int  ohs_batch_join(ohs_batch *b, void *hip_stream);
diff --git a/open_headstage_amd/_ffi.py b/open_headstage_amd/_ffi.py
--- a/open_headstage_amd/_ffi.py
+++ b/open_headstage_amd/_ffi.py
@@ -122,6 +122,7 @@
     "ohs_batch_process_scheduled_streams": (C.c_int, [vp, vp, vp, C.c_size_t, C.c_size_t, C.c_size_t, C.c_size_t,
                                                     C.POINTER(C.c_uint32), C.c_size_t, fp, C.c_size_t, vp]),
     "ohs_batch_last_eq_form": (C.c_int, [vp, C.POINTER(C.c_int), C.POINTER(C.c_int)]),
+    "ohs_batch_overlap_plan": (C.c_int, [C.c_size_t, C.c_int, C.POINTER(C.c_size_t), C.c_size_t, C.POINTER(C.c_size_t)]),
     "ohs_batch_join": (C.c_int, [vp, vp]),
     "ohs_batch_sync": (C.c_int, [vp, vp]),
     "ohs_batch_process_host": (C.c_int, [vp, vp, vp, C.c_size_t, C.c_size_t, C.c_size_t, C.c_size_t]),
diff --git a/open_headstage_amd/csrc/api_batch.hip b/open_headstage_amd/csrc/api_batch.hip
--- a/open_headstage_amd/csrc/api_batch.hip
+++ b/open_headstage_amd/csrc/api_batch.hip
@@ -340,8 +340,10 @@
         if (rc) return rc;
         return span_end(st);
     }
-    const std::vector<double> &kCut = tuning().overlap_cuts;
-    const int nch = (b->overlap && n_blocks >= 64) ? (int)kCut.size() - 1 : 1;
+    const OverlapPlan plan = (b->overlap && n_blocks >= 64)
+        ? overlap_plan(n_blocks, eq_pass_takes_wave_ring(ss, cs, (long long)frames, (int)b->eq.chains, 1, b->eq.exact_specials), tuning())
+        : OverlapPlan();
+    const int nch = plan.n;
     struct XcdScope {
         ohs_batch *b;
         XcdScope(ohs_batch *b_, int x) : b(b_)
@@ -352,8 +354,8 @@
     } xcd_scope(b, nch > 1 ? b->xcd_split : 0);
     bool joined = false;
     for (int i = 0; i < nch; ++i) {
-        const size_t blk0 = nch == 1 ? 0 : (size_t)(kCut[i] * (double)n_blocks);
-        const size_t blk1 = nch == 1 ? n_blocks : (i == nch - 1 ? n_blocks : (size_t)(kCut[i + 1] * (double)n_blocks));
+        const size_t blk0 = nch == 1 ? 0 : plan.cut[i];
+        const size_t blk1 = nch == 1 ? n_blocks : plan.cut[i + 1];
         const size_t off = blk0 * BS;
         const int nb_i = (int)(blk1 - blk0);
         if (nb_i <= 0) {
@@ -451,6 +453,17 @@
     if (n_tables > ((size_t)1 << 24)) return fail(OHS_ERR_INVALID_ARG, "n_tables too large");
     HIP_TRY(hipSetDevice(b->device));
     return eq_set_schedule_tables(b->eq, n_tables, coeffs, enabled, b->st);
+}
+
+int ohs_batch_overlap_plan(size_t n_blocks, int wave_ring, size_t *cuts, size_t cap, size_t *n_chunks)
+{
+    if (!cuts || !n_chunks) return fail(OHS_ERR_INVALID_ARG, "NULL argument");
+    const OverlapPlan plan = n_blocks >= 64 ? overlap_plan(n_blocks, wave_ring != 0, tuning()) : OverlapPlan();
+    if (cap < (size_t)plan.n + 1) return fail(OHS_ERR_INVALID_ARG, "cuts holds fewer than n_chunks + 1 entries");
+    for (int i = 0; i < plan.n; ++i) cuts[i] = plan.cut[i];
+    cuts[plan.n] = n_blocks;
+    *n_chunks = (size_t)plan.n;
+    return OHS_OK;
 }
 
 int ohs_batch_last_eq_form(const ohs_batch *b, int *form, int *scheduled)
diff --git a/open_headstage_amd/csrc/eq_quad_ring_asm.inc b/open_headstage_amd/csrc/eq_quad_ring_asm.inc
--- a/open_headstage_amd/csrc/eq_quad_ring_asm.inc
+++ b/open_headstage_amd/csrc/eq_quad_ring_asm.inc
@@ -1,7 +1,9 @@
 #define EQ_QUAD_RING_K 8
-#define EQ_QUAD_RING_LOOP \
+#define EQ_QUAD_RING_RUN \
     "s_mov_b32 vcc_lo, -1\n" \
     "s_mov_b32 vcc_hi, 0x3333ffff\n" \
+    "s_cmp_eq_u32 %[cnt], 0\n" \
+    "s_cbranch_scc1 3f\n" \
     ".p2align 5\n" \
     "1:\n" \
     "v_add_f32_dpp v3, v4, v5 wave_ror:1 row_mask:0xf bank_mask:0xf\n" \
@@ -653,5 +655,588 @@
     "v_mul_f32_dpp v6, v2, v7 quad_perm:[0,0,3,3] row_mask:0xf bank_mask:0xf\n" \
     "v_sub_f32_dpp v5, v2, v6 quad_perm:[0,0,1,2] row_mask:0xf bank_mask:0xf\n" \
     "s_cbranch_scc0 1b\n" \
+    "3:\n" \
+    "s_cmp_eq_u32 %[rem], 0\n" \
+    "s_cbranch_scc1 2f\n" \
+    "v_add_f32_dpp v3, v4, v5 wave_ror:1 row_mask:0xf bank_mask:0xf\n" \
+    "v_mul_f32_dpp v4, v2, v8 quad_perm:[0,0,0,3] row_mask:0xf bank_mask:0xf\n" \
+    "v_nop_e64\n" \
+    "v_mul_f32_dpp v6, v3, v7 quad_perm:[0,0,3,3] row_mask:0xf bank_mask:0xf\n" \
+    "v_sub_f32_dpp v5, v3, v6 quad_perm:[0,0,1,2] row_mask:0xf bank_mask:0xf\n" \
+    "v_add_f32_dpp v2, v4, v5 wave_ror:1 row_mask:0xf bank_mask:0xf\n" \
+    "v_mul_f32_dpp v4, v3, v8 quad_perm:[0,0,0,3] row_mask:0xf bank_mask:0xf\n" \
+    "v_nop_e64\n" \
+    "v_mul_f32_dpp v6, v2, v7 quad_perm:[0,0,3,3] row_mask:0xf bank_mask:0xf\n" \
+    "v_sub_f32_dpp v5, v2, v6 quad_perm:[0,0,1,2] row_mask:0xf bank_mask:0xf\n" \
+    "v_add_f32_dpp v3, v4, v5 wave_ror:1 row_mask:0xf bank_mask:0xf\n" \
+    "v_mul_f32_dpp v4, v2, v8 quad_perm:[0,0,0,3] row_mask:0xf bank_mask:0xf\n" \
+    "v_nop_e64\n" \
+    "v_mul_f32_dpp v6, v3, v7 quad_perm:[0,0,3,3] row_mask:0xf bank_mask:0xf\n" \
+    "v_sub_f32_dpp v5, v3, v6 quad_perm:[0,0,1,2] row_mask:0xf bank_mask:0xf\n" \
+    "v_add_f32_dpp v2, v4, v5 wave_ror:1 row_mask:0xf bank_mask:0xf\n" \
+    "v_mul_f32_dpp v4, v3, v8 quad_perm:[0,0,0,3] row_mask:0xf bank_mask:0xf\n" \
+    "v_nop_e64\n" \
+    "v_mul_f32_dpp v6, v2, v7 quad_perm:[0,0,3,3] row_mask:0xf bank_mask:0xf\n" \
+    "v_sub_f32_dpp v5, v2, v6 quad_perm:[0,0,1,2] row_mask:0xf bank_mask:0xf\n" \
+    "v_add_f32_dpp v3, v4, v5 wave_ror:1 row_mask:0xf bank_mask:0xf\n" \
+    "v_mul_f32_dpp v4, v2, v8 quad_perm:[0,0,0,3] row_mask:0xf bank_mask:0xf\n" \
+    "v_nop_e64\n" \
+    "v_mul_f32_dpp v6, v3, v7 quad_perm:[0,0,3,3] row_mask:0xf bank_mask:0xf\n" \
+    "v_sub_f32_dpp v5, v3, v6 quad_perm:[0,0,1,2] row_mask:0xf bank_mask:0xf\n" \
+    "v_add_f32_dpp v2, v4, v5 wave_ror:1 row_mask:0xf bank_mask:0xf\n" \
+    "v_mul_f32_dpp v4, v3, v8 quad_perm:[0,0,0,3] row_mask:0xf bank_mask:0xf\n" \
+    "v_nop_e64\n" \
+    "v_mul_f32_dpp v6, v2, v7 quad_perm:[0,0,3,3] row_mask:0xf bank_mask:0xf\n" \
+    "v_sub_f32_dpp v5, v2, v6 quad_perm:[0,0,1,2] row_mask:0xf bank_mask:0xf\n" \
+    "v_add_f32_dpp v3, v4, v5 wave_ror:1 row_mask:0xf bank_mask:0xf\n" \
+    "v_mul_f32_dpp v4, v2, v8 quad_perm:[0,0,0,3] row_mask:0xf bank_mask:0xf\n" \
+    "v_nop_e64\n" \
+    "v_mul_f32_dpp v6, v3, v7 quad_perm:[0,0,3,3] row_mask:0xf bank_mask:0xf\n" \
+    "v_sub_f32_dpp v5, v3, v6 quad_perm:[0,0,1,2] row_mask:0xf bank_mask:0xf\n" \
+    "v_add_f32_dpp v2, v4, v5 wave_ror:1 row_mask:0xf bank_mask:0xf\n" \
+    "v_mul_f32_dpp v4, v3, v8 quad_perm:[0,0,0,3] row_mask:0xf bank_mask:0xf\n" \
+    "buffer_store_dword v2, v0, %[rout], 0 offen offset:64\n" \
+    "v_mul_f32_dpp v6, v2, v7 quad_perm:[0,0,3,3] row_mask:0xf bank_mask:0xf\n" \
+    "v_sub_f32_dpp v5, v2, v6 quad_perm:[0,0,1,2] row_mask:0xf bank_mask:0xf\n" \
+    "v_add_f32_dpp v3, v4, v5 wave_ror:1 row_mask:0xf bank_mask:0xf\n" \
+    "v_mul_f32_dpp v4, v2, v8 quad_perm:[0,0,0,3] row_mask:0xf bank_mask:0xf\n" \
+    "v_cndmask_b32_dpp v4, v11, v4, vcc quad_perm:[0,1,0,1] row_mask:0xf bank_mask:0xf\n" \
+    "v_mul_f32_dpp v6, v3, v7 quad_perm:[0,0,3,3] row_mask:0xf bank_mask:0xf\n" \
+    "v_sub_f32_dpp v5, v3, v6 quad_perm:[0,0,1,2] row_mask:0xf bank_mask:0xf\n" \
+    "v_add_f32_dpp v2, v4, v5 wave_ror:1 row_mask:0xf bank_mask:0xf\n" \
+    "v_mul_f32_dpp v4, v3, v8 quad_perm:[0,0,0,3] row_mask:0xf bank_mask:0xf\n" \
+    "buffer_load_dword v11, v1, %[rin], 0 offen offset:512\n" \
+    "v_mul_f32_dpp v6, v2, v7 quad_perm:[0,0,3,3] row_mask:0xf bank_mask:0xf\n" \
+    "v_sub_f32_dpp v5, v2, v6 quad_perm:[0,0,1,2] row_mask:0xf bank_mask:0xf\n" \
+    "v_add_f32_dpp v3, v4, v5 wave_ror:1 row_mask:0xf bank_mask:0xf\n" \
+    "v_mul_f32_dpp v4, v2, v8 quad_perm:[0,0,0,3] row_mask:0xf bank_mask:0xf\n" \
+    "v_nop_e64\n" \
+    "v_mul_f32_dpp v6, v3, v7 quad_perm:[0,0,3,3] row_mask:0xf bank_mask:0xf\n" \
+    "v_sub_f32_dpp v5, v3, v6 quad_perm:[0,0,1,2] row_mask:0xf bank_mask:0xf\n" \
+    "v_add_f32_dpp v2, v4, v5 wave_ror:1 row_mask:0xf bank_mask:0xf\n" \
+    "v_mul_f32_dpp v4, v3, v8 quad_perm:[0,0,0,3] row_mask:0xf bank_mask:0xf\n" \
+    "v_nop_e64\n" \
+    "v_mul_f32_dpp v6, v2, v7 quad_perm:[0,0,3,3] row_mask:0xf bank_mask:0xf\n" \
+    "v_sub_f32_dpp v5, v2, v6 quad_perm:[0,0,1,2] row_mask:0xf bank_mask:0xf\n" \
+    "v_add_f32_dpp v3, v4, v5 wave_ror:1 row_mask:0xf bank_mask:0xf\n" \
+    "v_mul_f32_dpp v4, v2, v8 quad_perm:[0,0,0,3] row_mask:0xf bank_mask:0xf\n" \
+    "v_nop_e64\n" \
+    "v_mul_f32_dpp v6, v3, v7 quad_perm:[0,0,3,3] row_mask:0xf bank_mask:0xf\n" \
+    "v_sub_f32_dpp v5, v3, v6 quad_perm:[0,0,1,2] row_mask:0xf bank_mask:0xf\n" \
+    "v_add_f32_dpp v2, v4, v5 wave_ror:1 row_mask:0xf bank_mask:0xf\n" \
+    "v_mul_f32_dpp v4, v3, v8 quad_perm:[0,0,0,3] row_mask:0xf bank_mask:0xf\n" \
+    "s_waitcnt vmcnt(21)\n" \
+    "s_cmp_eq_u32 %[rem], 1\n" \
+    "v_mul_f32_dpp v6, v2, v7 quad_perm:[0,0,3,3] row_mask:0xf bank_mask:0xf\n" \
+    "v_sub_f32_dpp v5, v2, v6 quad_perm:[0,0,1,2] row_mask:0xf bank_mask:0xf\n" \
+    "v_add_f32_dpp v3, v4, v5 wave_ror:1 row_mask:0xf bank_mask:0xf\n" \
+    "v_mul_f32_dpp v4, v2, v8 quad_perm:[0,0,0,3] row_mask:0xf bank_mask:0xf\n" \
+    "buffer_store_dword v3, v0, %[rout], 0 offen offset:92\n" \
+    "v_mul_f32_dpp v6, v3, v7 quad_perm:[0,0,3,3] row_mask:0xf bank_mask:0xf\n" \
+    "v_sub_f32_dpp v5, v3, v6 quad_perm:[0,0,1,2] row_mask:0xf bank_mask:0xf\n" \
+    "v_add_f32_dpp v2, v4, v5 wave_ror:1 row_mask:0xf bank_mask:0xf\n" \
+    "v_mul_f32_dpp v4, v3, v8 quad_perm:[0,0,0,3] row_mask:0xf bank_mask:0xf\n" \
+    "v_cndmask_b32_dpp v4, v12, v4, vcc quad_perm:[0,1,2,3] row_mask:0xf bank_mask:0xf\n" \
+    "v_mul_f32_dpp v6, v2, v7 quad_perm:[0,0,3,3] row_mask:0xf bank_mask:0xf\n" \
+    "v_sub_f32_dpp v5, v2, v6 quad_perm:[0,0,1,2] row_mask:0xf bank_mask:0xf\n" \
+    "s_cbranch_scc1 2f\n" \
+    "s_nop 0\n" \
+    "v_add_f32_dpp v3, v4, v5 wave_ror:1 row_mask:0xf bank_mask:0xf\n" \
+    "v_mul_f32_dpp v4, v2, v8 quad_perm:[0,0,0,3] row_mask:0xf bank_mask:0xf\n" \
+    "v_nop_e64\n" \
+    "v_mul_f32_dpp v6, v3, v7 quad_perm:[0,0,3,3] row_mask:0xf bank_mask:0xf\n" \
+    "v_sub_f32_dpp v5, v3, v6 quad_perm:[0,0,1,2] row_mask:0xf bank_mask:0xf\n" \
+    "v_add_f32_dpp v2, v4, v5 wave_ror:1 row_mask:0xf bank_mask:0xf\n" \
+    "v_mul_f32_dpp v4, v3, v8 quad_perm:[0,0,0,3] row_mask:0xf bank_mask:0xf\n" \
+    "v_nop_e64\n" \
+    "v_mul_f32_dpp v6, v2, v7 quad_perm:[0,0,3,3] row_mask:0xf bank_mask:0xf\n" \
+    "v_sub_f32_dpp v5, v2, v6 quad_perm:[0,0,1,2] row_mask:0xf bank_mask:0xf\n" \
+    "v_add_f32_dpp v3, v4, v5 wave_ror:1 row_mask:0xf bank_mask:0xf\n" \
+    "v_mul_f32_dpp v4, v2, v8 quad_perm:[0,0,0,3] row_mask:0xf bank_mask:0xf\n" \
+    "v_nop_e64\n" \
+    "v_mul_f32_dpp v6, v3, v7 quad_perm:[0,0,3,3] row_mask:0xf bank_mask:0xf\n" \
+    "v_sub_f32_dpp v5, v3, v6 quad_perm:[0,0,1,2] row_mask:0xf bank_mask:0xf\n" \
+    "v_add_f32_dpp v2, v4, v5 wave_ror:1 row_mask:0xf bank_mask:0xf\n" \
+    "v_mul_f32_dpp v4, v3, v8 quad_perm:[0,0,0,3] row_mask:0xf bank_mask:0xf\n" \
+    "v_nop_e64\n" \
+    "v_mul_f32_dpp v6, v2, v7 quad_perm:[0,0,3,3] row_mask:0xf bank_mask:0xf\n" \
+    "v_sub_f32_dpp v5, v2, v6 quad_perm:[0,0,1,2] row_mask:0xf bank_mask:0xf\n" \
+    "v_add_f32_dpp v3, v4, v5 wave_ror:1 row_mask:0xf bank_mask:0xf\n" \
+    "v_mul_f32_dpp v4, v2, v8 quad_perm:[0,0,0,3] row_mask:0xf bank_mask:0xf\n" \
+    "v_nop_e64\n" \
+    "v_mul_f32_dpp v6, v3, v7 quad_perm:[0,0,3,3] row_mask:0xf bank_mask:0xf\n" \
+    "v_sub_f32_dpp v5, v3, v6 quad_perm:[0,0,1,2] row_mask:0xf bank_mask:0xf\n" \
+    "v_add_f32_dpp v2, v4, v5 wave_ror:1 row_mask:0xf bank_mask:0xf\n" \
+    "v_mul_f32_dpp v4, v3, v8 quad_perm:[0,0,0,3] row_mask:0xf bank_mask:0xf\n" \
+    "v_nop_e64\n" \
+    "v_mul_f32_dpp v6, v2, v7 quad_perm:[0,0,3,3] row_mask:0xf bank_mask:0xf\n" \
+    "v_sub_f32_dpp v5, v2, v6 quad_perm:[0,0,1,2] row_mask:0xf bank_mask:0xf\n" \
+    "v_add_f32_dpp v3, v4, v5 wave_ror:1 row_mask:0xf bank_mask:0xf\n" \
+    "v_mul_f32_dpp v4, v2, v8 quad_perm:[0,0,0,3] row_mask:0xf bank_mask:0xf\n" \
+    "v_nop_e64\n" \
+    "v_mul_f32_dpp v6, v3, v7 quad_perm:[0,0,3,3] row_mask:0xf bank_mask:0xf\n" \
+    "v_sub_f32_dpp v5, v3, v6 quad_perm:[0,0,1,2] row_mask:0xf bank_mask:0xf\n" \
+    "v_add_f32_dpp v2, v4, v5 wave_ror:1 row_mask:0xf bank_mask:0xf\n" \
+    "v_mul_f32_dpp v4, v3, v8 quad_perm:[0,0,0,3] row_mask:0xf bank_mask:0xf\n" \
+    "buffer_store_dword v2, v0, %[rout], 0 offen offset:128\n" \
+    "v_mul_f32_dpp v6, v2, v7 quad_perm:[0,0,3,3] row_mask:0xf bank_mask:0xf\n" \
+    "v_sub_f32_dpp v5, v2, v6 quad_perm:[0,0,1,2] row_mask:0xf bank_mask:0xf\n" \
+    "v_add_f32_dpp v3, v4, v5 wave_ror:1 row_mask:0xf bank_mask:0xf\n" \
+    "v_mul_f32_dpp v4, v2, v8 quad_perm:[0,0,0,3] row_mask:0xf bank_mask:0xf\n" \
+    "v_cndmask_b32_dpp v4, v12, v4, vcc quad_perm:[0,1,0,1] row_mask:0xf bank_mask:0xf\n" \
+    "v_mul_f32_dpp v6, v3, v7 quad_perm:[0,0,3,3] row_mask:0xf bank_mask:0xf\n" \
+    "v_sub_f32_dpp v5, v3, v6 quad_perm:[0,0,1,2] row_mask:0xf bank_mask:0xf\n" \
+    "v_add_f32_dpp v2, v4, v5 wave_ror:1 row_mask:0xf bank_mask:0xf\n" \
+    "v_mul_f32_dpp v4, v3, v8 quad_perm:[0,0,0,3] row_mask:0xf bank_mask:0xf\n" \
+    "buffer_load_dword v12, v1, %[rin], 0 offen offset:576\n" \
+    "v_mul_f32_dpp v6, v2, v7 quad_perm:[0,0,3,3] row_mask:0xf bank_mask:0xf\n" \
+    "v_sub_f32_dpp v5, v2, v6 quad_perm:[0,0,1,2] row_mask:0xf bank_mask:0xf\n" \
+    "v_add_f32_dpp v3, v4, v5 wave_ror:1 row_mask:0xf bank_mask:0xf\n" \
+    "v_mul_f32_dpp v4, v2, v8 quad_perm:[0,0,0,3] row_mask:0xf bank_mask:0xf\n" \
+    "v_nop_e64\n" \
+    "v_mul_f32_dpp v6, v3, v7 quad_perm:[0,0,3,3] row_mask:0xf bank_mask:0xf\n" \
+    "v_sub_f32_dpp v5, v3, v6 quad_perm:[0,0,1,2] row_mask:0xf bank_mask:0xf\n" \
+    "v_add_f32_dpp v2, v4, v5 wave_ror:1 row_mask:0xf bank_mask:0xf\n" \
+    "v_mul_f32_dpp v4, v3, v8 quad_perm:[0,0,0,3] row_mask:0xf bank_mask:0xf\n" \
+    "v_nop_e64\n" \
+    "v_mul_f32_dpp v6, v2, v7 quad_perm:[0,0,3,3] row_mask:0xf bank_mask:0xf\n" \
+    "v_sub_f32_dpp v5, v2, v6 quad_perm:[0,0,1,2] row_mask:0xf bank_mask:0xf\n" \
+    "v_add_f32_dpp v3, v4, v5 wave_ror:1 row_mask:0xf bank_mask:0xf\n" \
+    "v_mul_f32_dpp v4, v2, v8 quad_perm:[0,0,0,3] row_mask:0xf bank_mask:0xf\n" \
+    "v_nop_e64\n" \
+    "v_mul_f32_dpp v6, v3, v7 quad_perm:[0,0,3,3] row_mask:0xf bank_mask:0xf\n" \
+    "v_sub_f32_dpp v5, v3, v6 quad_perm:[0,0,1,2] row_mask:0xf bank_mask:0xf\n" \
+    "v_add_f32_dpp v2, v4, v5 wave_ror:1 row_mask:0xf bank_mask:0xf\n" \
+    "v_mul_f32_dpp v4, v3, v8 quad_perm:[0,0,0,3] row_mask:0xf bank_mask:0xf\n" \
+    "s_waitcnt vmcnt(21)\n" \
+    "s_cmp_eq_u32 %[rem], 2\n" \
+    "v_mul_f32_dpp v6, v2, v7 quad_perm:[0,0,3,3] row_mask:0xf bank_mask:0xf\n" \
+    "v_sub_f32_dpp v5, v2, v6 quad_perm:[0,0,1,2] row_mask:0xf bank_mask:0xf\n" \
+    "v_add_f32_dpp v3, v4, v5 wave_ror:1 row_mask:0xf bank_mask:0xf\n" \
+    "v_mul_f32_dpp v4, v2, v8 quad_perm:[0,0,0,3] row_mask:0xf bank_mask:0xf\n" \
+    "buffer_store_dword v3, v0, %[rout], 0 offen offset:156\n" \
+    "v_mul_f32_dpp v6, v3, v7 quad_perm:[0,0,3,3] row_mask:0xf bank_mask:0xf\n" \
+    "v_sub_f32_dpp v5, v3, v6 quad_perm:[0,0,1,2] row_mask:0xf bank_mask:0xf\n" \
+    "v_add_f32_dpp v2, v4, v5 wave_ror:1 row_mask:0xf bank_mask:0xf\n" \
+    "v_mul_f32_dpp v4, v3, v8 quad_perm:[0,0,0,3] row_mask:0xf bank_mask:0xf\n" \
+    "v_cndmask_b32_dpp v4, v13, v4, vcc quad_perm:[0,1,2,3] row_mask:0xf bank_mask:0xf\n" \
+    "v_mul_f32_dpp v6, v2, v7 quad_perm:[0,0,3,3] row_mask:0xf bank_mask:0xf\n" \
+    "v_sub_f32_dpp v5, v2, v6 quad_perm:[0,0,1,2] row_mask:0xf bank_mask:0xf\n" \
+    "s_cbranch_scc1 2f\n" \
+    "s_nop 0\n" \
+    "v_add_f32_dpp v3, v4, v5 wave_ror:1 row_mask:0xf bank_mask:0xf\n" \
+    "v_mul_f32_dpp v4, v2, v8 quad_perm:[0,0,0,3] row_mask:0xf bank_mask:0xf\n" \
+    "v_nop_e64\n" \
+    "v_mul_f32_dpp v6, v3, v7 quad_perm:[0,0,3,3] row_mask:0xf bank_mask:0xf\n" \
+    "v_sub_f32_dpp v5, v3, v6 quad_perm:[0,0,1,2] row_mask:0xf bank_mask:0xf\n" \
+    "v_add_f32_dpp v2, v4, v5 wave_ror:1 row_mask:0xf bank_mask:0xf\n" \
+    "v_mul_f32_dpp v4, v3, v8 quad_perm:[0,0,0,3] row_mask:0xf bank_mask:0xf\n" \
+    "v_nop_e64\n" \
+    "v_mul_f32_dpp v6, v2, v7 quad_perm:[0,0,3,3] row_mask:0xf bank_mask:0xf\n" \
+    "v_sub_f32_dpp v5, v2, v6 quad_perm:[0,0,1,2] row_mask:0xf bank_mask:0xf\n" \
+    "v_add_f32_dpp v3, v4, v5 wave_ror:1 row_mask:0xf bank_mask:0xf\n" \
+    "v_mul_f32_dpp v4, v2, v8 quad_perm:[0,0,0,3] row_mask:0xf bank_mask:0xf\n" \
+    "v_nop_e64\n" \
+    "v_mul_f32_dpp v6, v3, v7 quad_perm:[0,0,3,3] row_mask:0xf bank_mask:0xf\n" \
+    "v_sub_f32_dpp v5, v3, v6 quad_perm:[0,0,1,2] row_mask:0xf bank_mask:0xf\n" \
+    "v_add_f32_dpp v2, v4, v5 wave_ror:1 row_mask:0xf bank_mask:0xf\n" \
+    "v_mul_f32_dpp v4, v3, v8 quad_perm:[0,0,0,3] row_mask:0xf bank_mask:0xf\n" \
+    "v_nop_e64\n" \
+    "v_mul_f32_dpp v6, v2, v7 quad_perm:[0,0,3,3] row_mask:0xf bank_mask:0xf\n" \
+    "v_sub_f32_dpp v5, v2, v6 quad_perm:[0,0,1,2] row_mask:0xf bank_mask:0xf\n" \
+    "v_add_f32_dpp v3, v4, v5 wave_ror:1 row_mask:0xf bank_mask:0xf\n" \
+    "v_mul_f32_dpp v4, v2, v8 quad_perm:[0,0,0,3] row_mask:0xf bank_mask:0xf\n" \
+    "v_nop_e64\n" \
+    "v_mul_f32_dpp v6, v3, v7 quad_perm:[0,0,3,3] row_mask:0xf bank_mask:0xf\n" \
+    "v_sub_f32_dpp v5, v3, v6 quad_perm:[0,0,1,2] row_mask:0xf bank_mask:0xf\n" \
+    "v_add_f32_dpp v2, v4, v5 wave_ror:1 row_mask:0xf bank_mask:0xf\n" \
+    "v_mul_f32_dpp v4, v3, v8 quad_perm:[0,0,0,3] row_mask:0xf bank_mask:0xf\n" \
+    "v_nop_e64\n" \
+    "v_mul_f32_dpp v6, v2, v7 quad_perm:[0,0,3,3] row_mask:0xf bank_mask:0xf\n" \
+    "v_sub_f32_dpp v5, v2, v6 quad_perm:[0,0,1,2] row_mask:0xf bank_mask:0xf\n" \
+    "v_add_f32_dpp v3, v4, v5 wave_ror:1 row_mask:0xf bank_mask:0xf\n" \
+    "v_mul_f32_dpp v4, v2, v8 quad_perm:[0,0,0,3] row_mask:0xf bank_mask:0xf\n" \
+    "v_nop_e64\n" \
+    "v_mul_f32_dpp v6, v3, v7 quad_perm:[0,0,3,3] row_mask:0xf bank_mask:0xf\n" \
+    "v_sub_f32_dpp v5, v3, v6 quad_perm:[0,0,1,2] row_mask:0xf bank_mask:0xf\n" \
+    "v_add_f32_dpp v2, v4, v5 wave_ror:1 row_mask:0xf bank_mask:0xf\n" \
+    "v_mul_f32_dpp v4, v3, v8 quad_perm:[0,0,0,3] row_mask:0xf bank_mask:0xf\n" \
+    "buffer_store_dword v2, v0, %[rout], 0 offen offset:192\n" \
+    "v_mul_f32_dpp v6, v2, v7 quad_perm:[0,0,3,3] row_mask:0xf bank_mask:0xf\n" \
+    "v_sub_f32_dpp v5, v2, v6 quad_perm:[0,0,1,2] row_mask:0xf bank_mask:0xf\n" \
+    "v_add_f32_dpp v3, v4, v5 wave_ror:1 row_mask:0xf bank_mask:0xf\n" \
+    "v_mul_f32_dpp v4, v2, v8 quad_perm:[0,0,0,3] row_mask:0xf bank_mask:0xf\n" \
+    "v_cndmask_b32_dpp v4, v13, v4, vcc quad_perm:[0,1,0,1] row_mask:0xf bank_mask:0xf\n" \
+    "v_mul_f32_dpp v6, v3, v7 quad_perm:[0,0,3,3] row_mask:0xf bank_mask:0xf\n" \
+    "v_sub_f32_dpp v5, v3, v6 quad_perm:[0,0,1,2] row_mask:0xf bank_mask:0xf\n" \
+    "v_add_f32_dpp v2, v4, v5 wave_ror:1 row_mask:0xf bank_mask:0xf\n" \
+    "v_mul_f32_dpp v4, v3, v8 quad_perm:[0,0,0,3] row_mask:0xf bank_mask:0xf\n" \
+    "buffer_load_dword v13, v1, %[rin], 0 offen offset:640\n" \
+    "v_mul_f32_dpp v6, v2, v7 quad_perm:[0,0,3,3] row_mask:0xf bank_mask:0xf\n" \
+    "v_sub_f32_dpp v5, v2, v6 quad_perm:[0,0,1,2] row_mask:0xf bank_mask:0xf\n" \
+    "v_add_f32_dpp v3, v4, v5 wave_ror:1 row_mask:0xf bank_mask:0xf\n" \
+    "v_mul_f32_dpp v4, v2, v8 quad_perm:[0,0,0,3] row_mask:0xf bank_mask:0xf\n" \
+    "v_nop_e64\n" \
+    "v_mul_f32_dpp v6, v3, v7 quad_perm:[0,0,3,3] row_mask:0xf bank_mask:0xf\n" \
+    "v_sub_f32_dpp v5, v3, v6 quad_perm:[0,0,1,2] row_mask:0xf bank_mask:0xf\n" \
+    "v_add_f32_dpp v2, v4, v5 wave_ror:1 row_mask:0xf bank_mask:0xf\n" \
+    "v_mul_f32_dpp v4, v3, v8 quad_perm:[0,0,0,3] row_mask:0xf bank_mask:0xf\n" \
+    "v_nop_e64\n" \
+    "v_mul_f32_dpp v6, v2, v7 quad_perm:[0,0,3,3] row_mask:0xf bank_mask:0xf\n" \
+    "v_sub_f32_dpp v5, v2, v6 quad_perm:[0,0,1,2] row_mask:0xf bank_mask:0xf\n" \
+    "v_add_f32_dpp v3, v4, v5 wave_ror:1 row_mask:0xf bank_mask:0xf\n" \
+    "v_mul_f32_dpp v4, v2, v8 quad_perm:[0,0,0,3] row_mask:0xf bank_mask:0xf\n" \
+    "v_nop_e64\n" \
+    "v_mul_f32_dpp v6, v3, v7 quad_perm:[0,0,3,3] row_mask:0xf bank_mask:0xf\n" \
+    "v_sub_f32_dpp v5, v3, v6 quad_perm:[0,0,1,2] row_mask:0xf bank_mask:0xf\n" \
+    "v_add_f32_dpp v2, v4, v5 wave_ror:1 row_mask:0xf bank_mask:0xf\n" \
+    "v_mul_f32_dpp v4, v3, v8 quad_perm:[0,0,0,3] row_mask:0xf bank_mask:0xf\n" \
+    "s_waitcnt vmcnt(21)\n" \
+    "s_cmp_eq_u32 %[rem], 3\n" \
+    "v_mul_f32_dpp v6, v2, v7 quad_perm:[0,0,3,3] row_mask:0xf bank_mask:0xf\n" \
+    "v_sub_f32_dpp v5, v2, v6 quad_perm:[0,0,1,2] row_mask:0xf bank_mask:0xf\n" \
+    "v_add_f32_dpp v3, v4, v5 wave_ror:1 row_mask:0xf bank_mask:0xf\n" \
+    "v_mul_f32_dpp v4, v2, v8 quad_perm:[0,0,0,3] row_mask:0xf bank_mask:0xf\n" \
+    "buffer_store_dword v3, v0, %[rout], 0 offen offset:220\n" \
+    "v_mul_f32_dpp v6, v3, v7 quad_perm:[0,0,3,3] row_mask:0xf bank_mask:0xf\n" \
+    "v_sub_f32_dpp v5, v3, v6 quad_perm:[0,0,1,2] row_mask:0xf bank_mask:0xf\n" \
+    "v_add_f32_dpp v2, v4, v5 wave_ror:1 row_mask:0xf bank_mask:0xf\n" \
+    "v_mul_f32_dpp v4, v3, v8 quad_perm:[0,0,0,3] row_mask:0xf bank_mask:0xf\n" \
+    "v_cndmask_b32_dpp v4, v14, v4, vcc quad_perm:[0,1,2,3] row_mask:0xf bank_mask:0xf\n" \
+    "v_mul_f32_dpp v6, v2, v7 quad_perm:[0,0,3,3] row_mask:0xf bank_mask:0xf\n" \
+    "v_sub_f32_dpp v5, v2, v6 quad_perm:[0,0,1,2] row_mask:0xf bank_mask:0xf\n" \
+    "s_cbranch_scc1 2f\n" \
+    "s_nop 0\n" \
+    "v_add_f32_dpp v3, v4, v5 wave_ror:1 row_mask:0xf bank_mask:0xf\n" \
+    "v_mul_f32_dpp v4, v2, v8 quad_perm:[0,0,0,3] row_mask:0xf bank_mask:0xf\n" \
+    "v_nop_e64\n" \
+    "v_mul_f32_dpp v6, v3, v7 quad_perm:[0,0,3,3] row_mask:0xf bank_mask:0xf\n" \
+    "v_sub_f32_dpp v5, v3, v6 quad_perm:[0,0,1,2] row_mask:0xf bank_mask:0xf\n" \
+    "v_add_f32_dpp v2, v4, v5 wave_ror:1 row_mask:0xf bank_mask:0xf\n" \
+    "v_mul_f32_dpp v4, v3, v8 quad_perm:[0,0,0,3] row_mask:0xf bank_mask:0xf\n" \
+    "v_nop_e64\n" \
+    "v_mul_f32_dpp v6, v2, v7 quad_perm:[0,0,3,3] row_mask:0xf bank_mask:0xf\n" \
+    "v_sub_f32_dpp v5, v2, v6 quad_perm:[0,0,1,2] row_mask:0xf bank_mask:0xf\n" \
+    "v_add_f32_dpp v3, v4, v5 wave_ror:1 row_mask:0xf bank_mask:0xf\n" \
+    "v_mul_f32_dpp v4, v2, v8 quad_perm:[0,0,0,3] row_mask:0xf bank_mask:0xf\n" \
+    "v_nop_e64\n" \
+    "v_mul_f32_dpp v6, v3, v7 quad_perm:[0,0,3,3] row_mask:0xf bank_mask:0xf\n" \
+    "v_sub_f32_dpp v5, v3, v6 quad_perm:[0,0,1,2] row_mask:0xf bank_mask:0xf\n" \
+    "v_add_f32_dpp v2, v4, v5 wave_ror:1 row_mask:0xf bank_mask:0xf\n" \
+    "v_mul_f32_dpp v4, v3, v8 quad_perm:[0,0,0,3] row_mask:0xf bank_mask:0xf\n" \
+    "v_nop_e64\n" \
+    "v_mul_f32_dpp v6, v2, v7 quad_perm:[0,0,3,3] row_mask:0xf bank_mask:0xf\n" \
+    "v_sub_f32_dpp v5, v2, v6 quad_perm:[0,0,1,2] row_mask:0xf bank_mask:0xf\n" \
+    "v_add_f32_dpp v3, v4, v5 wave_ror:1 row_mask:0xf bank_mask:0xf\n" \
+    "v_mul_f32_dpp v4, v2, v8 quad_perm:[0,0,0,3] row_mask:0xf bank_mask:0xf\n" \
+    "v_nop_e64\n" \
+    "v_mul_f32_dpp v6, v3, v7 quad_perm:[0,0,3,3] row_mask:0xf bank_mask:0xf\n" \
+    "v_sub_f32_dpp v5, v3, v6 quad_perm:[0,0,1,2] row_mask:0xf bank_mask:0xf\n" \
+    "v_add_f32_dpp v2, v4, v5 wave_ror:1 row_mask:0xf bank_mask:0xf\n" \
+    "v_mul_f32_dpp v4, v3, v8 quad_perm:[0,0,0,3] row_mask:0xf bank_mask:0xf\n" \
+    "v_nop_e64\n" \
+    "v_mul_f32_dpp v6, v2, v7 quad_perm:[0,0,3,3] row_mask:0xf bank_mask:0xf\n" \
+    "v_sub_f32_dpp v5, v2, v6 quad_perm:[0,0,1,2] row_mask:0xf bank_mask:0xf\n" \
+    "v_add_f32_dpp v3, v4, v5 wave_ror:1 row_mask:0xf bank_mask:0xf\n" \
+    "v_mul_f32_dpp v4, v2, v8 quad_perm:[0,0,0,3] row_mask:0xf bank_mask:0xf\n" \
+    "v_nop_e64\n" \
+    "v_mul_f32_dpp v6, v3, v7 quad_perm:[0,0,3,3] row_mask:0xf bank_mask:0xf\n" \
+    "v_sub_f32_dpp v5, v3, v6 quad_perm:[0,0,1,2] row_mask:0xf bank_mask:0xf\n" \
+    "v_add_f32_dpp v2, v4, v5 wave_ror:1 row_mask:0xf bank_mask:0xf\n" \
+    "v_mul_f32_dpp v4, v3, v8 quad_perm:[0,0,0,3] row_mask:0xf bank_mask:0xf\n" \
+    "buffer_store_dword v2, v0, %[rout], 0 offen offset:256\n" \
+    "v_mul_f32_dpp v6, v2, v7 quad_perm:[0,0,3,3] row_mask:0xf bank_mask:0xf\n" \
+    "v_sub_f32_dpp v5, v2, v6 quad_perm:[0,0,1,2] row_mask:0xf bank_mask:0xf\n" \
+    "v_add_f32_dpp v3, v4, v5 wave_ror:1 row_mask:0xf bank_mask:0xf\n" \
+    "v_mul_f32_dpp v4, v2, v8 quad_perm:[0,0,0,3] row_mask:0xf bank_mask:0xf\n" \
+    "v_cndmask_b32_dpp v4, v14, v4, vcc quad_perm:[0,1,0,1] row_mask:0xf bank_mask:0xf\n" \
+    "v_mul_f32_dpp v6, v3, v7 quad_perm:[0,0,3,3] row_mask:0xf bank_mask:0xf\n" \
+    "v_sub_f32_dpp v5, v3, v6 quad_perm:[0,0,1,2] row_mask:0xf bank_mask:0xf\n" \
+    "v_add_f32_dpp v2, v4, v5 wave_ror:1 row_mask:0xf bank_mask:0xf\n" \
+    "v_mul_f32_dpp v4, v3, v8 quad_perm:[0,0,0,3] row_mask:0xf bank_mask:0xf\n" \
+    "buffer_load_dword v14, v1, %[rin], 0 offen offset:704\n" \
+    "v_mul_f32_dpp v6, v2, v7 quad_perm:[0,0,3,3] row_mask:0xf bank_mask:0xf\n" \
+    "v_sub_f32_dpp v5, v2, v6 quad_perm:[0,0,1,2] row_mask:0xf bank_mask:0xf\n" \
+    "v_add_f32_dpp v3, v4, v5 wave_ror:1 row_mask:0xf bank_mask:0xf\n" \
+    "v_mul_f32_dpp v4, v2, v8 quad_perm:[0,0,0,3] row_mask:0xf bank_mask:0xf\n" \
+    "v_nop_e64\n" \
+    "v_mul_f32_dpp v6, v3, v7 quad_perm:[0,0,3,3] row_mask:0xf bank_mask:0xf\n" \
+    "v_sub_f32_dpp v5, v3, v6 quad_perm:[0,0,1,2] row_mask:0xf bank_mask:0xf\n" \
+    "v_add_f32_dpp v2, v4, v5 wave_ror:1 row_mask:0xf bank_mask:0xf\n" \
+    "v_mul_f32_dpp v4, v3, v8 quad_perm:[0,0,0,3] row_mask:0xf bank_mask:0xf\n" \
+    "v_nop_e64\n" \
+    "v_mul_f32_dpp v6, v2, v7 quad_perm:[0,0,3,3] row_mask:0xf bank_mask:0xf\n" \
+    "v_sub_f32_dpp v5, v2, v6 quad_perm:[0,0,1,2] row_mask:0xf bank_mask:0xf\n" \
+    "v_add_f32_dpp v3, v4, v5 wave_ror:1 row_mask:0xf bank_mask:0xf\n" \
+    "v_mul_f32_dpp v4, v2, v8 quad_perm:[0,0,0,3] row_mask:0xf bank_mask:0xf\n" \
+    "v_nop_e64\n" \
+    "v_mul_f32_dpp v6, v3, v7 quad_perm:[0,0,3,3] row_mask:0xf bank_mask:0xf\n" \
+    "v_sub_f32_dpp v5, v3, v6 quad_perm:[0,0,1,2] row_mask:0xf bank_mask:0xf\n" \
+    "v_add_f32_dpp v2, v4, v5 wave_ror:1 row_mask:0xf bank_mask:0xf\n" \
+    "v_mul_f32_dpp v4, v3, v8 quad_perm:[0,0,0,3] row_mask:0xf bank_mask:0xf\n" \
+    "s_waitcnt vmcnt(21)\n" \
+    "s_cmp_eq_u32 %[rem], 4\n" \
+    "v_mul_f32_dpp v6, v2, v7 quad_perm:[0,0,3,3] row_mask:0xf bank_mask:0xf\n" \
+    "v_sub_f32_dpp v5, v2, v6 quad_perm:[0,0,1,2] row_mask:0xf bank_mask:0xf\n" \
+    "v_add_f32_dpp v3, v4, v5 wave_ror:1 row_mask:0xf bank_mask:0xf\n" \
+    "v_mul_f32_dpp v4, v2, v8 quad_perm:[0,0,0,3] row_mask:0xf bank_mask:0xf\n" \
+    "buffer_store_dword v3, v0, %[rout], 0 offen offset:284\n" \
+    "v_mul_f32_dpp v6, v3, v7 quad_perm:[0,0,3,3] row_mask:0xf bank_mask:0xf\n" \
+    "v_sub_f32_dpp v5, v3, v6 quad_perm:[0,0,1,2] row_mask:0xf bank_mask:0xf\n" \
+    "v_add_f32_dpp v2, v4, v5 wave_ror:1 row_mask:0xf bank_mask:0xf\n" \
+    "v_mul_f32_dpp v4, v3, v8 quad_perm:[0,0,0,3] row_mask:0xf bank_mask:0xf\n" \
+    "v_cndmask_b32_dpp v4, v15, v4, vcc quad_perm:[0,1,2,3] row_mask:0xf bank_mask:0xf\n" \
+    "v_mul_f32_dpp v6, v2, v7 quad_perm:[0,0,3,3] row_mask:0xf bank_mask:0xf\n" \
+    "v_sub_f32_dpp v5, v2, v6 quad_perm:[0,0,1,2] row_mask:0xf bank_mask:0xf\n" \
+    "s_cbranch_scc1 2f\n" \
+    "s_nop 0\n" \
+    "v_add_f32_dpp v3, v4, v5 wave_ror:1 row_mask:0xf bank_mask:0xf\n" \
+    "v_mul_f32_dpp v4, v2, v8 quad_perm:[0,0,0,3] row_mask:0xf bank_mask:0xf\n" \
+    "v_nop_e64\n" \
+    "v_mul_f32_dpp v6, v3, v7 quad_perm:[0,0,3,3] row_mask:0xf bank_mask:0xf\n" \
+    "v_sub_f32_dpp v5, v3, v6 quad_perm:[0,0,1,2] row_mask:0xf bank_mask:0xf\n" \
+    "v_add_f32_dpp v2, v4, v5 wave_ror:1 row_mask:0xf bank_mask:0xf\n" \
+    "v_mul_f32_dpp v4, v3, v8 quad_perm:[0,0,0,3] row_mask:0xf bank_mask:0xf\n" \
+    "v_nop_e64\n" \
+    "v_mul_f32_dpp v6, v2, v7 quad_perm:[0,0,3,3] row_mask:0xf bank_mask:0xf\n" \
+    "v_sub_f32_dpp v5, v2, v6 quad_perm:[0,0,1,2] row_mask:0xf bank_mask:0xf\n" \
+    "v_add_f32_dpp v3, v4, v5 wave_ror:1 row_mask:0xf bank_mask:0xf\n" \
+    "v_mul_f32_dpp v4, v2, v8 quad_perm:[0,0,0,3] row_mask:0xf bank_mask:0xf\n" \
+    "v_nop_e64\n" \
+    "v_mul_f32_dpp v6, v3, v7 quad_perm:[0,0,3,3] row_mask:0xf bank_mask:0xf\n" \
+    "v_sub_f32_dpp v5, v3, v6 quad_perm:[0,0,1,2] row_mask:0xf bank_mask:0xf\n" \
+    "v_add_f32_dpp v2, v4, v5 wave_ror:1 row_mask:0xf bank_mask:0xf\n" \
+    "v_mul_f32_dpp v4, v3, v8 quad_perm:[0,0,0,3] row_mask:0xf bank_mask:0xf\n" \
+    "v_nop_e64\n" \
+    "v_mul_f32_dpp v6, v2, v7 quad_perm:[0,0,3,3] row_mask:0xf bank_mask:0xf\n" \
+    "v_sub_f32_dpp v5, v2, v6 quad_perm:[0,0,1,2] row_mask:0xf bank_mask:0xf\n" \
+    "v_add_f32_dpp v3, v4, v5 wave_ror:1 row_mask:0xf bank_mask:0xf\n" \
+    "v_mul_f32_dpp v4, v2, v8 quad_perm:[0,0,0,3] row_mask:0xf bank_mask:0xf\n" \
+    "v_nop_e64\n" \
+    "v_mul_f32_dpp v6, v3, v7 quad_perm:[0,0,3,3] row_mask:0xf bank_mask:0xf\n" \
+    "v_sub_f32_dpp v5, v3, v6 quad_perm:[0,0,1,2] row_mask:0xf bank_mask:0xf\n" \
+    "v_add_f32_dpp v2, v4, v5 wave_ror:1 row_mask:0xf bank_mask:0xf\n" \
+    "v_mul_f32_dpp v4, v3, v8 quad_perm:[0,0,0,3] row_mask:0xf bank_mask:0xf\n" \
+    "v_nop_e64\n" \
+    "v_mul_f32_dpp v6, v2, v7 quad_perm:[0,0,3,3] row_mask:0xf bank_mask:0xf\n" \
+    "v_sub_f32_dpp v5, v2, v6 quad_perm:[0,0,1,2] row_mask:0xf bank_mask:0xf\n" \
+    "v_add_f32_dpp v3, v4, v5 wave_ror:1 row_mask:0xf bank_mask:0xf\n" \
+    "v_mul_f32_dpp v4, v2, v8 quad_perm:[0,0,0,3] row_mask:0xf bank_mask:0xf\n" \
+    "v_nop_e64\n" \
+    "v_mul_f32_dpp v6, v3, v7 quad_perm:[0,0,3,3] row_mask:0xf bank_mask:0xf\n" \
+    "v_sub_f32_dpp v5, v3, v6 quad_perm:[0,0,1,2] row_mask:0xf bank_mask:0xf\n" \
+    "v_add_f32_dpp v2, v4, v5 wave_ror:1 row_mask:0xf bank_mask:0xf\n" \
+    "v_mul_f32_dpp v4, v3, v8 quad_perm:[0,0,0,3] row_mask:0xf bank_mask:0xf\n" \
+    "buffer_store_dword v2, v0, %[rout], 0 offen offset:320\n" \
+    "v_mul_f32_dpp v6, v2, v7 quad_perm:[0,0,3,3] row_mask:0xf bank_mask:0xf\n" \
+    "v_sub_f32_dpp v5, v2, v6 quad_perm:[0,0,1,2] row_mask:0xf bank_mask:0xf\n" \
+    "v_add_f32_dpp v3, v4, v5 wave_ror:1 row_mask:0xf bank_mask:0xf\n" \
+    "v_mul_f32_dpp v4, v2, v8 quad_perm:[0,0,0,3] row_mask:0xf bank_mask:0xf\n" \
+    "v_cndmask_b32_dpp v4, v15, v4, vcc quad_perm:[0,1,0,1] row_mask:0xf bank_mask:0xf\n" \
+    "v_mul_f32_dpp v6, v3, v7 quad_perm:[0,0,3,3] row_mask:0xf bank_mask:0xf\n" \
+    "v_sub_f32_dpp v5, v3, v6 quad_perm:[0,0,1,2] row_mask:0xf bank_mask:0xf\n" \
+    "v_add_f32_dpp v2, v4, v5 wave_ror:1 row_mask:0xf bank_mask:0xf\n" \
+    "v_mul_f32_dpp v4, v3, v8 quad_perm:[0,0,0,3] row_mask:0xf bank_mask:0xf\n" \
+    "buffer_load_dword v15, v1, %[rin], 0 offen offset:768\n" \
+    "v_mul_f32_dpp v6, v2, v7 quad_perm:[0,0,3,3] row_mask:0xf bank_mask:0xf\n" \
+    "v_sub_f32_dpp v5, v2, v6 quad_perm:[0,0,1,2] row_mask:0xf bank_mask:0xf\n" \
+    "v_add_f32_dpp v3, v4, v5 wave_ror:1 row_mask:0xf bank_mask:0xf\n" \
+    "v_mul_f32_dpp v4, v2, v8 quad_perm:[0,0,0,3] row_mask:0xf bank_mask:0xf\n" \
+    "v_nop_e64\n" \
+    "v_mul_f32_dpp v6, v3, v7 quad_perm:[0,0,3,3] row_mask:0xf bank_mask:0xf\n" \
+    "v_sub_f32_dpp v5, v3, v6 quad_perm:[0,0,1,2] row_mask:0xf bank_mask:0xf\n" \
+    "v_add_f32_dpp v2, v4, v5 wave_ror:1 row_mask:0xf bank_mask:0xf\n" \
+    "v_mul_f32_dpp v4, v3, v8 quad_perm:[0,0,0,3] row_mask:0xf bank_mask:0xf\n" \
+    "v_nop_e64\n" \
+    "v_mul_f32_dpp v6, v2, v7 quad_perm:[0,0,3,3] row_mask:0xf bank_mask:0xf\n" \
+    "v_sub_f32_dpp v5, v2, v6 quad_perm:[0,0,1,2] row_mask:0xf bank_mask:0xf\n" \
+    "v_add_f32_dpp v3, v4, v5 wave_ror:1 row_mask:0xf bank_mask:0xf\n" \
+    "v_mul_f32_dpp v4, v2, v8 quad_perm:[0,0,0,3] row_mask:0xf bank_mask:0xf\n" \
+    "v_nop_e64\n" \
+    "v_mul_f32_dpp v6, v3, v7 quad_perm:[0,0,3,3] row_mask:0xf bank_mask:0xf\n" \
+    "v_sub_f32_dpp v5, v3, v6 quad_perm:[0,0,1,2] row_mask:0xf bank_mask:0xf\n" \
+    "v_add_f32_dpp v2, v4, v5 wave_ror:1 row_mask:0xf bank_mask:0xf\n" \
+    "v_mul_f32_dpp v4, v3, v8 quad_perm:[0,0,0,3] row_mask:0xf bank_mask:0xf\n" \
+    "s_waitcnt vmcnt(21)\n" \
+    "s_cmp_eq_u32 %[rem], 5\n" \
+    "v_mul_f32_dpp v6, v2, v7 quad_perm:[0,0,3,3] row_mask:0xf bank_mask:0xf\n" \
+    "v_sub_f32_dpp v5, v2, v6 quad_perm:[0,0,1,2] row_mask:0xf bank_mask:0xf\n" \
+    "v_add_f32_dpp v3, v4, v5 wave_ror:1 row_mask:0xf bank_mask:0xf\n" \
+    "v_mul_f32_dpp v4, v2, v8 quad_perm:[0,0,0,3] row_mask:0xf bank_mask:0xf\n" \
+    "buffer_store_dword v3, v0, %[rout], 0 offen offset:348\n" \
+    "v_mul_f32_dpp v6, v3, v7 quad_perm:[0,0,3,3] row_mask:0xf bank_mask:0xf\n" \
+    "v_sub_f32_dpp v5, v3, v6 quad_perm:[0,0,1,2] row_mask:0xf bank_mask:0xf\n" \
+    "v_add_f32_dpp v2, v4, v5 wave_ror:1 row_mask:0xf bank_mask:0xf\n" \
+    "v_mul_f32_dpp v4, v3, v8 quad_perm:[0,0,0,3] row_mask:0xf bank_mask:0xf\n" \
+    "v_cndmask_b32_dpp v4, v16, v4, vcc quad_perm:[0,1,2,3] row_mask:0xf bank_mask:0xf\n" \
+    "v_mul_f32_dpp v6, v2, v7 quad_perm:[0,0,3,3] row_mask:0xf bank_mask:0xf\n" \
+    "v_sub_f32_dpp v5, v2, v6 quad_perm:[0,0,1,2] row_mask:0xf bank_mask:0xf\n" \
+    "s_cbranch_scc1 2f\n" \
+    "s_nop 0\n" \
+    "v_add_f32_dpp v3, v4, v5 wave_ror:1 row_mask:0xf bank_mask:0xf\n" \
+    "v_mul_f32_dpp v4, v2, v8 quad_perm:[0,0,0,3] row_mask:0xf bank_mask:0xf\n" \
+    "v_nop_e64\n" \
+    "v_mul_f32_dpp v6, v3, v7 quad_perm:[0,0,3,3] row_mask:0xf bank_mask:0xf\n" \
+    "v_sub_f32_dpp v5, v3, v6 quad_perm:[0,0,1,2] row_mask:0xf bank_mask:0xf\n" \
+    "v_add_f32_dpp v2, v4, v5 wave_ror:1 row_mask:0xf bank_mask:0xf\n" \
+    "v_mul_f32_dpp v4, v3, v8 quad_perm:[0,0,0,3] row_mask:0xf bank_mask:0xf\n" \
+    "v_nop_e64\n" \
+    "v_mul_f32_dpp v6, v2, v7 quad_perm:[0,0,3,3] row_mask:0xf bank_mask:0xf\n" \
+    "v_sub_f32_dpp v5, v2, v6 quad_perm:[0,0,1,2] row_mask:0xf bank_mask:0xf\n" \
+    "v_add_f32_dpp v3, v4, v5 wave_ror:1 row_mask:0xf bank_mask:0xf\n" \
+    "v_mul_f32_dpp v4, v2, v8 quad_perm:[0,0,0,3] row_mask:0xf bank_mask:0xf\n" \
+    "v_nop_e64\n" \
+    "v_mul_f32_dpp v6, v3, v7 quad_perm:[0,0,3,3] row_mask:0xf bank_mask:0xf\n" \
+    "v_sub_f32_dpp v5, v3, v6 quad_perm:[0,0,1,2] row_mask:0xf bank_mask:0xf\n" \
+    "v_add_f32_dpp v2, v4, v5 wave_ror:1 row_mask:0xf bank_mask:0xf\n" \
+    "v_mul_f32_dpp v4, v3, v8 quad_perm:[0,0,0,3] row_mask:0xf bank_mask:0xf\n" \
+    "v_nop_e64\n" \
+    "v_mul_f32_dpp v6, v2, v7 quad_perm:[0,0,3,3] row_mask:0xf bank_mask:0xf\n" \
+    "v_sub_f32_dpp v5, v2, v6 quad_perm:[0,0,1,2] row_mask:0xf bank_mask:0xf\n" \
+    "v_add_f32_dpp v3, v4, v5 wave_ror:1 row_mask:0xf bank_mask:0xf\n" \
+    "v_mul_f32_dpp v4, v2, v8 quad_perm:[0,0,0,3] row_mask:0xf bank_mask:0xf\n" \
+    "v_nop_e64\n" \
+    "v_mul_f32_dpp v6, v3, v7 quad_perm:[0,0,3,3] row_mask:0xf bank_mask:0xf\n" \
+    "v_sub_f32_dpp v5, v3, v6 quad_perm:[0,0,1,2] row_mask:0xf bank_mask:0xf\n" \
+    "v_add_f32_dpp v2, v4, v5 wave_ror:1 row_mask:0xf bank_mask:0xf\n" \
+    "v_mul_f32_dpp v4, v3, v8 quad_perm:[0,0,0,3] row_mask:0xf bank_mask:0xf\n" \
+    "v_nop_e64\n" \
+    "v_mul_f32_dpp v6, v2, v7 quad_perm:[0,0,3,3] row_mask:0xf bank_mask:0xf\n" \
+    "v_sub_f32_dpp v5, v2, v6 quad_perm:[0,0,1,2] row_mask:0xf bank_mask:0xf\n" \
+    "v_add_f32_dpp v3, v4, v5 wave_ror:1 row_mask:0xf bank_mask:0xf\n" \
+    "v_mul_f32_dpp v4, v2, v8 quad_perm:[0,0,0,3] row_mask:0xf bank_mask:0xf\n" \
+    "v_nop_e64\n" \
+    "v_mul_f32_dpp v6, v3, v7 quad_perm:[0,0,3,3] row_mask:0xf bank_mask:0xf\n" \
+    "v_sub_f32_dpp v5, v3, v6 quad_perm:[0,0,1,2] row_mask:0xf bank_mask:0xf\n" \
+    "v_add_f32_dpp v2, v4, v5 wave_ror:1 row_mask:0xf bank_mask:0xf\n" \
+    "v_mul_f32_dpp v4, v3, v8 quad_perm:[0,0,0,3] row_mask:0xf bank_mask:0xf\n" \
+    "buffer_store_dword v2, v0, %[rout], 0 offen offset:384\n" \
+    "v_mul_f32_dpp v6, v2, v7 quad_perm:[0,0,3,3] row_mask:0xf bank_mask:0xf\n" \
+    "v_sub_f32_dpp v5, v2, v6 quad_perm:[0,0,1,2] row_mask:0xf bank_mask:0xf\n" \
+    "v_add_f32_dpp v3, v4, v5 wave_ror:1 row_mask:0xf bank_mask:0xf\n" \
+    "v_mul_f32_dpp v4, v2, v8 quad_perm:[0,0,0,3] row_mask:0xf bank_mask:0xf\n" \
+    "v_cndmask_b32_dpp v4, v16, v4, vcc quad_perm:[0,1,0,1] row_mask:0xf bank_mask:0xf\n" \
+    "v_mul_f32_dpp v6, v3, v7 quad_perm:[0,0,3,3] row_mask:0xf bank_mask:0xf\n" \
+    "v_sub_f32_dpp v5, v3, v6 quad_perm:[0,0,1,2] row_mask:0xf bank_mask:0xf\n" \
+    "v_add_f32_dpp v2, v4, v5 wave_ror:1 row_mask:0xf bank_mask:0xf\n" \
+    "v_mul_f32_dpp v4, v3, v8 quad_perm:[0,0,0,3] row_mask:0xf bank_mask:0xf\n" \
+    "buffer_load_dword v16, v1, %[rin], 0 offen offset:832\n" \
+    "v_mul_f32_dpp v6, v2, v7 quad_perm:[0,0,3,3] row_mask:0xf bank_mask:0xf\n" \
+    "v_sub_f32_dpp v5, v2, v6 quad_perm:[0,0,1,2] row_mask:0xf bank_mask:0xf\n" \
+    "v_add_f32_dpp v3, v4, v5 wave_ror:1 row_mask:0xf bank_mask:0xf\n" \
+    "v_mul_f32_dpp v4, v2, v8 quad_perm:[0,0,0,3] row_mask:0xf bank_mask:0xf\n" \
+    "v_nop_e64\n" \
+    "v_mul_f32_dpp v6, v3, v7 quad_perm:[0,0,3,3] row_mask:0xf bank_mask:0xf\n" \
+    "v_sub_f32_dpp v5, v3, v6 quad_perm:[0,0,1,2] row_mask:0xf bank_mask:0xf\n" \
+    "v_add_f32_dpp v2, v4, v5 wave_ror:1 row_mask:0xf bank_mask:0xf\n" \
+    "v_mul_f32_dpp v4, v3, v8 quad_perm:[0,0,0,3] row_mask:0xf bank_mask:0xf\n" \
+    "v_nop_e64\n" \
+    "v_mul_f32_dpp v6, v2, v7 quad_perm:[0,0,3,3] row_mask:0xf bank_mask:0xf\n" \
+    "v_sub_f32_dpp v5, v2, v6 quad_perm:[0,0,1,2] row_mask:0xf bank_mask:0xf\n" \
+    "v_add_f32_dpp v3, v4, v5 wave_ror:1 row_mask:0xf bank_mask:0xf\n" \
+    "v_mul_f32_dpp v4, v2, v8 quad_perm:[0,0,0,3] row_mask:0xf bank_mask:0xf\n" \
+    "v_nop_e64\n" \
+    "v_mul_f32_dpp v6, v3, v7 quad_perm:[0,0,3,3] row_mask:0xf bank_mask:0xf\n" \
+    "v_sub_f32_dpp v5, v3, v6 quad_perm:[0,0,1,2] row_mask:0xf bank_mask:0xf\n" \
+    "v_add_f32_dpp v2, v4, v5 wave_ror:1 row_mask:0xf bank_mask:0xf\n" \
+    "v_mul_f32_dpp v4, v3, v8 quad_perm:[0,0,0,3] row_mask:0xf bank_mask:0xf\n" \
+    "s_waitcnt vmcnt(21)\n" \
+    "s_cmp_eq_u32 %[rem], 6\n" \
+    "v_mul_f32_dpp v6, v2, v7 quad_perm:[0,0,3,3] row_mask:0xf bank_mask:0xf\n" \
+    "v_sub_f32_dpp v5, v2, v6 quad_perm:[0,0,1,2] row_mask:0xf bank_mask:0xf\n" \
+    "v_add_f32_dpp v3, v4, v5 wave_ror:1 row_mask:0xf bank_mask:0xf\n" \
+    "v_mul_f32_dpp v4, v2, v8 quad_perm:[0,0,0,3] row_mask:0xf bank_mask:0xf\n" \
+    "buffer_store_dword v3, v0, %[rout], 0 offen offset:412\n" \
+    "v_mul_f32_dpp v6, v3, v7 quad_perm:[0,0,3,3] row_mask:0xf bank_mask:0xf\n" \
+    "v_sub_f32_dpp v5, v3, v6 quad_perm:[0,0,1,2] row_mask:0xf bank_mask:0xf\n" \
+    "v_add_f32_dpp v2, v4, v5 wave_ror:1 row_mask:0xf bank_mask:0xf\n" \
+    "v_mul_f32_dpp v4, v3, v8 quad_perm:[0,0,0,3] row_mask:0xf bank_mask:0xf\n" \
+    "v_cndmask_b32_dpp v4, v17, v4, vcc quad_perm:[0,1,2,3] row_mask:0xf bank_mask:0xf\n" \
+    "v_mul_f32_dpp v6, v2, v7 quad_perm:[0,0,3,3] row_mask:0xf bank_mask:0xf\n" \
+    "v_sub_f32_dpp v5, v2, v6 quad_perm:[0,0,1,2] row_mask:0xf bank_mask:0xf\n" \
+    "s_cbranch_scc1 2f\n" \
+    "s_nop 0\n" \
+    "v_add_f32_dpp v3, v4, v5 wave_ror:1 row_mask:0xf bank_mask:0xf\n" \
+    "v_mul_f32_dpp v4, v2, v8 quad_perm:[0,0,0,3] row_mask:0xf bank_mask:0xf\n" \
+    "v_nop_e64\n" \
+    "v_mul_f32_dpp v6, v3, v7 quad_perm:[0,0,3,3] row_mask:0xf bank_mask:0xf\n" \
+    "v_sub_f32_dpp v5, v3, v6 quad_perm:[0,0,1,2] row_mask:0xf bank_mask:0xf\n" \
+    "v_add_f32_dpp v2, v4, v5 wave_ror:1 row_mask:0xf bank_mask:0xf\n" \
+    "v_mul_f32_dpp v4, v3, v8 quad_perm:[0,0,0,3] row_mask:0xf bank_mask:0xf\n" \
+    "v_nop_e64\n" \
+    "v_mul_f32_dpp v6, v2, v7 quad_perm:[0,0,3,3] row_mask:0xf bank_mask:0xf\n" \
+    "v_sub_f32_dpp v5, v2, v6 quad_perm:[0,0,1,2] row_mask:0xf bank_mask:0xf\n" \
+    "v_add_f32_dpp v3, v4, v5 wave_ror:1 row_mask:0xf bank_mask:0xf\n" \
+    "v_mul_f32_dpp v4, v2, v8 quad_perm:[0,0,0,3] row_mask:0xf bank_mask:0xf\n" \
+    "v_nop_e64\n" \
+    "v_mul_f32_dpp v6, v3, v7 quad_perm:[0,0,3,3] row_mask:0xf bank_mask:0xf\n" \
+    "v_sub_f32_dpp v5, v3, v6 quad_perm:[0,0,1,2] row_mask:0xf bank_mask:0xf\n" \
+    "v_add_f32_dpp v2, v4, v5 wave_ror:1 row_mask:0xf bank_mask:0xf\n" \
+    "v_mul_f32_dpp v4, v3, v8 quad_perm:[0,0,0,3] row_mask:0xf bank_mask:0xf\n" \
+    "v_nop_e64\n" \
+    "v_mul_f32_dpp v6, v2, v7 quad_perm:[0,0,3,3] row_mask:0xf bank_mask:0xf\n" \
+    "v_sub_f32_dpp v5, v2, v6 quad_perm:[0,0,1,2] row_mask:0xf bank_mask:0xf\n" \
+    "v_add_f32_dpp v3, v4, v5 wave_ror:1 row_mask:0xf bank_mask:0xf\n" \
+    "v_mul_f32_dpp v4, v2, v8 quad_perm:[0,0,0,3] row_mask:0xf bank_mask:0xf\n" \
+    "v_nop_e64\n" \
+    "v_mul_f32_dpp v6, v3, v7 quad_perm:[0,0,3,3] row_mask:0xf bank_mask:0xf\n" \
+    "v_sub_f32_dpp v5, v3, v6 quad_perm:[0,0,1,2] row_mask:0xf bank_mask:0xf\n" \
+    "v_add_f32_dpp v2, v4, v5 wave_ror:1 row_mask:0xf bank_mask:0xf\n" \
+    "v_mul_f32_dpp v4, v3, v8 quad_perm:[0,0,0,3] row_mask:0xf bank_mask:0xf\n" \
+    "v_nop_e64\n" \
+    "v_mul_f32_dpp v6, v2, v7 quad_perm:[0,0,3,3] row_mask:0xf bank_mask:0xf\n" \
+    "v_sub_f32_dpp v5, v2, v6 quad_perm:[0,0,1,2] row_mask:0xf bank_mask:0xf\n" \
+    "v_add_f32_dpp v3, v4, v5 wave_ror:1 row_mask:0xf bank_mask:0xf\n" \
+    "v_mul_f32_dpp v4, v2, v8 quad_perm:[0,0,0,3] row_mask:0xf bank_mask:0xf\n" \
+    "v_nop_e64\n" \
+    "v_mul_f32_dpp v6, v3, v7 quad_perm:[0,0,3,3] row_mask:0xf bank_mask:0xf\n" \
+    "v_sub_f32_dpp v5, v3, v6 quad_perm:[0,0,1,2] row_mask:0xf bank_mask:0xf\n" \
+    "v_add_f32_dpp v2, v4, v5 wave_ror:1 row_mask:0xf bank_mask:0xf\n" \
+    "v_mul_f32_dpp v4, v3, v8 quad_perm:[0,0,0,3] row_mask:0xf bank_mask:0xf\n" \
+    "buffer_store_dword v2, v0, %[rout], 0 offen offset:448\n" \
+    "v_mul_f32_dpp v6, v2, v7 quad_perm:[0,0,3,3] row_mask:0xf bank_mask:0xf\n" \
+    "v_sub_f32_dpp v5, v2, v6 quad_perm:[0,0,1,2] row_mask:0xf bank_mask:0xf\n" \
+    "v_add_f32_dpp v3, v4, v5 wave_ror:1 row_mask:0xf bank_mask:0xf\n" \
+    "v_mul_f32_dpp v4, v2, v8 quad_perm:[0,0,0,3] row_mask:0xf bank_mask:0xf\n" \
+    "v_cndmask_b32_dpp v4, v17, v4, vcc quad_perm:[0,1,0,1] row_mask:0xf bank_mask:0xf\n" \
+    "v_mul_f32_dpp v6, v3, v7 quad_perm:[0,0,3,3] row_mask:0xf bank_mask:0xf\n" \
+    "v_sub_f32_dpp v5, v3, v6 quad_perm:[0,0,1,2] row_mask:0xf bank_mask:0xf\n" \
+    "v_add_f32_dpp v2, v4, v5 wave_ror:1 row_mask:0xf bank_mask:0xf\n" \
+    "v_mul_f32_dpp v4, v3, v8 quad_perm:[0,0,0,3] row_mask:0xf bank_mask:0xf\n" \
+    "buffer_load_dword v17, v1, %[rin], 0 offen offset:896\n" \
+    "v_mul_f32_dpp v6, v2, v7 quad_perm:[0,0,3,3] row_mask:0xf bank_mask:0xf\n" \
+    "v_sub_f32_dpp v5, v2, v6 quad_perm:[0,0,1,2] row_mask:0xf bank_mask:0xf\n" \
+    "v_add_f32_dpp v3, v4, v5 wave_ror:1 row_mask:0xf bank_mask:0xf\n" \
+    "v_mul_f32_dpp v4, v2, v8 quad_perm:[0,0,0,3] row_mask:0xf bank_mask:0xf\n" \
+    "v_nop_e64\n" \
+    "v_mul_f32_dpp v6, v3, v7 quad_perm:[0,0,3,3] row_mask:0xf bank_mask:0xf\n" \
+    "v_sub_f32_dpp v5, v3, v6 quad_perm:[0,0,1,2] row_mask:0xf bank_mask:0xf\n" \
+    "v_add_f32_dpp v2, v4, v5 wave_ror:1 row_mask:0xf bank_mask:0xf\n" \
+    "v_mul_f32_dpp v4, v3, v8 quad_perm:[0,0,0,3] row_mask:0xf bank_mask:0xf\n" \
+    "v_nop_e64\n" \
+    "v_mul_f32_dpp v6, v2, v7 quad_perm:[0,0,3,3] row_mask:0xf bank_mask:0xf\n" \
+    "v_sub_f32_dpp v5, v2, v6 quad_perm:[0,0,1,2] row_mask:0xf bank_mask:0xf\n" \
+    "v_add_f32_dpp v3, v4, v5 wave_ror:1 row_mask:0xf bank_mask:0xf\n" \
+    "v_mul_f32_dpp v4, v2, v8 quad_perm:[0,0,0,3] row_mask:0xf bank_mask:0xf\n" \
+    "v_nop_e64\n" \
+    "v_mul_f32_dpp v6, v3, v7 quad_perm:[0,0,3,3] row_mask:0xf bank_mask:0xf\n" \
+    "v_sub_f32_dpp v5, v3, v6 quad_perm:[0,0,1,2] row_mask:0xf bank_mask:0xf\n" \
+    "v_add_f32_dpp v2, v4, v5 wave_ror:1 row_mask:0xf bank_mask:0xf\n" \
+    "v_mul_f32_dpp v4, v3, v8 quad_perm:[0,0,0,3] row_mask:0xf bank_mask:0xf\n" \
+    "s_waitcnt vmcnt(21)\n" \
+    "s_nop 0\n" \
+    "v_mul_f32_dpp v6, v2, v7 quad_perm:[0,0,3,3] row_mask:0xf bank_mask:0xf\n" \
+    "v_sub_f32_dpp v5, v2, v6 quad_perm:[0,0,1,2] row_mask:0xf bank_mask:0xf\n" \
+    "v_add_f32_dpp v3, v4, v5 wave_ror:1 row_mask:0xf bank_mask:0xf\n" \
+    "v_mul_f32_dpp v4, v2, v8 quad_perm:[0,0,0,3] row_mask:0xf bank_mask:0xf\n" \
+    "buffer_store_dword v3, v0, %[rout], 0 offen offset:476\n" \
+    "v_mul_f32_dpp v6, v3, v7 quad_perm:[0,0,3,3] row_mask:0xf bank_mask:0xf\n" \
+    "v_sub_f32_dpp v5, v3, v6 quad_perm:[0,0,1,2] row_mask:0xf bank_mask:0xf\n" \
+    "v_add_f32_dpp v2, v4, v5 wave_ror:1 row_mask:0xf bank_mask:0xf\n" \
+    "v_mul_f32_dpp v4, v3, v8 quad_perm:[0,0,0,3] row_mask:0xf bank_mask:0xf\n" \
+    "v_cndmask_b32_dpp v4, v18, v4, vcc quad_perm:[0,1,2,3] row_mask:0xf bank_mask:0xf\n" \
+    "v_mul_f32_dpp v6, v2, v7 quad_perm:[0,0,3,3] row_mask:0xf bank_mask:0xf\n" \
+    "v_sub_f32_dpp v5, v2, v6 quad_perm:[0,0,1,2] row_mask:0xf bank_mask:0xf\n" \
+    "2:\n" \
     "s_waitcnt vmcnt(0)\n" \
     "s_nop 1\n"
diff --git a/open_headstage_amd/csrc/eq_quad_ring_body.hpp b/open_headstage_amd/csrc/eq_quad_ring_body.hpp
--- a/open_headstage_amd/csrc/eq_quad_ring_body.hpp
+++ b/open_headstage_amd/csrc/eq_quad_ring_body.hpp
@@ -1,4 +1,6 @@
 #pragma once
+#include <type_traits>
+
 #include "kernels.h"
 #include "eq_ring64_body.hpp"
 #include "eq_quad_ring_asm.inc"
@@ -43,28 +45,28 @@
     QuadRegs r = {0.0f, 0.0f, 0.0f, 0.0f, 0.0f};
     float xcur = load_x(-1), xnext = load_x(0);
 
-    const int g_hi = (n32 + 1) / G;
-    const int iters = g_hi - 5 >= K ? (g_hi - 5) / K : 0;
-    const int g1 = iters ? g_hi : -1, g0 = iters ? g_hi - iters * K : -1;
+    const int g_hi = (n32 + 1) / G, g0 = 5;
+    const int n_asm = g_hi > g0 ? g_hi - g0 : 0, iters = n_asm / K, rem = n_asm % K;
     float x2 = 0.0f, x3 = 0.0f, x4 = 0.0f, x5 = 0.0f, x6 = 0.0f, x7 = 0.0f;
-    if (iters) {
+    if (n_asm) {
         x2 = load_x(g0 + 2); x3 = load_x(g0 + 3); x4 = load_x(g0 + 4);
         x5 = load_x(g0 + 5); x6 = load_x(g0 + 6); x7 = load_x(g0 + 7);
     }
 
     auto group_cpp = [&](int g) {
         const float xnext2 = load_x(g + 2);
-        auto step = [&](float &zc, const float zo, int s) {
+        auto step = [&](float &zc, const float zo, int s, auto port_) {
+            constexpr int port = decltype(port_)::value;
             const int stp = g * G + s;
             zc = dpp_mov<kWaveRor1>(r.Zp, r.Zp) + r.G;
             r.Zp = dpp_mov<kQp0003>(zo, zo) * C2;
-            if (s == 8 || s == 15) {
+            if constexpr (port == 1) {
                 const int yi = stp + ss;
                 if (st_lane && (unsigned)yi < (unsigned)n32) ring2_st(dst0, (unsigned)yi * 4u, zc);
-            } else if (s == 9) {
+            } else if constexpr (port == 2) {
                 const float xb = dpp_mov<kQp0101>(xcur, xcur);
                 r.Zp = inj_lane ? xb : r.Zp;
-            } else if (s == 16) {
+            } else if constexpr (port == 3) {
                 r.Zp = inj_lane ? xnext : r.Zp;
             }
             r.P = dpp_mov<kQp0033>(zc, zc) * C1;
@@ -72,36 +74,62 @@
             if (st_band && stp == t_in) r.G = s_init;
             if (st_band && stp == n32 + t_in) s_save = r.G;
         };
+        constexpr std::integral_constant<int, 0> none{};
+        constexpr std::integral_constant<int, 1> store{};
+        constexpr std::integral_constant<int, 2> inject_b{};
+        constexpr std::integral_constant<int, 3> inject_a{};
+        auto plain_pairs = [&](int s0, int s1) {
 #pragma unroll 1
-        for (int s = 1; s <= G; s += 2) {
-            step(r.Z1, r.Z0, s);
-            step(r.Z0, r.Z1, s + 1);
-        }
+            for (int s = s0; s < s1; s += 2) {
+                step(r.Z1, r.Z0, s, none);
+                step(r.Z0, r.Z1, s + 1, none);
+            }
+        };
+        plain_pairs(1, 7);
+        step(r.Z1, r.Z0, 7, none);
+        step(r.Z0, r.Z1, 8, store);
+        step(r.Z1, r.Z0, 9, inject_b);
+        step(r.Z0, r.Z1, 10, none);
+        plain_pairs(11, 15);
+        step(r.Z1, r.Z0, 15, store);
+        step(r.Z0, r.Z1, 16, inject_a);
         xcur = xnext;
         xnext = xnext2;
     };
 
     const int g_total = (n32 + 62 + G - 1) / G;
     int g = -1;
-    const int head_end = iters ? g0 : g_total;
+    const int head_end = n_asm ? g0 : g_total;
 #pragma unroll 1
     for (; g < head_end; ++g) group_cpp(g);
-    if (iters) {
+    if (n_asm) {
         const unsigned bytes = (unsigned)n32 * 4u;
         const ring64_rsrc_t rin = ring64_rsrc(src0, bytes), rout = ring64_rsrc(dst0, bytes);
         unsigned voff_st = st_lane ? (unsigned)(G * (g0 - 1) + 8 + ss) * 4u : 0xFFFFF000u;
         unsigned voff_ld = conv ? (unsigned)(G * g0 + xs) * 4u : 0xFFFFF000u;
         const unsigned inc_ld = conv ? 4u * G * K : 0u, inc_st = st_lane ? 4u * G * K : 0u;
         unsigned cnt = 0u - (unsigned)__builtin_amdgcn_readfirstlane(iters);
+        const int rem_s = __builtin_amdgcn_readfirstlane(rem);
         asm volatile(
             "s_nop 4\n"
-            EQ_QUAD_RING_LOOP
+            EQ_QUAD_RING_RUN
             : [Z0] "+{v2}"(r.Z0), [Z1] "+{v3}"(r.Z1), [Zp] "+{v4}"(r.Zp), [Gr] "+{v5}"(r.G), [P] "+{v6}"(r.P),
               [vs] "+{v0}"(voff_st), [vl] "+{v1}"(voff_ld), [x0] "+{v11}"(xcur), [x1] "+{v12}"(xnext), [x2] "+{v13}"(x2),
               [x3] "+{v14}"(x3), [x4] "+{v15}"(x4), [x5] "+{v16}"(x5), [x6] "+{v17}"(x6), [x7] "+{v18}"(x7), [cnt] "+s"(cnt)
-            : [C1] "{v7}"(C1), [C2] "{v8}"(C2), [incl] "{v9}"(inc_ld), [incs] "{v10}"(inc_st), [rin] "s"(rin), [rout] "s"(rout)
+            : [C1] "{v7}"(C1), [C2] "{v8}"(C2), [incl] "{v9}"(inc_ld), [incs] "{v10}"(inc_st), [rin] "s"(rin), [rout] "s"(rout),
+              [rem] "s"(rem_s)
             : "memory", "scc", "vcc");
-        g = g1;
+        switch (rem_s) {
+        case 0: break;
+        case 1: xcur = xnext; xnext = x2; break;
+        case 2: xcur = x2; xnext = x3; break;
+        case 3: xcur = x3; xnext = x4; break;
+        case 4: xcur = x4; xnext = x5; break;
+        case 5: xcur = x5; xnext = x6; break;
+        case 6: xcur = x6; xnext = x7; break;
+        default: { const float x0 = xcur; xcur = x7; xnext = x0; } break;
+        }
+        g = g_hi;
 #pragma unroll 1
         for (; g < g_total; ++g) group_cpp(g);
     }
diff --git a/open_headstage_amd/csrc/tuning.cpp b/open_headstage_amd/csrc/tuning.cpp
--- a/open_headstage_amd/csrc/tuning.cpp
+++ b/open_headstage_amd/csrc/tuning.cpp
@@ -46,6 +46,60 @@
 #endif
 }
 
+OverlapPlan overlap_plan(size_t n_blocks, bool wave_ring, const Tuning &t)
+{
+    OverlapPlan p;
+    p.cut[1] = n_blocks;
+    if (t.overlap_cuts_forced || !wave_ring) {
+        const int n = std::min((int)t.overlap_cuts.size() - 1, OverlapPlan::kMaxChunks);
+        if (n < 2) return p;
+        p.n = n;
+        for (int i = 1; i < n; ++i) p.cut[i] = std::max(p.cut[i - 1], std::min(n_blocks, (size_t)(t.overlap_cuts[(size_t)i] * (double)n_blocks)));
+        p.cut[n] = n_blocks;
+        return p;
+    }
+    const size_t floor_b = (size_t)std::max(1, t.overlap_min_blocks);
+    const double ratio = std::min(0.25, std::max(1.0 / 64.0, t.overlap_ratio));
+    if (n_blocks < 2 * floor_b) return p;
+    if (t.overlap_tail_frac * (double)n_blocks < (double)floor_b) {
+        const int k_max = std::min((int)t.overlap_cuts.size() - 1, OverlapPlan::kMaxChunks);
+        const int k = (int)std::min<size_t>((size_t)std::max(k_max, 1), n_blocks / floor_b);
+        long long len[OverlapPlan::kMaxChunks];
+        if (k < k_max) {
+            for (int i = 1; i < k; ++i) len[i] = (long long)floor_b;
+            len[0] = (long long)n_blocks - (long long)floor_b * (k - 1);
+        } else {
+            size_t at = 0;
+            for (int i = 0; i < k; ++i) {
+                const size_t to = i == k - 1 ? n_blocks : std::max(at, (size_t)(t.overlap_cuts[(size_t)i + 1] * (double)n_blocks));
+                len[i] = (long long)(to - at);
+                at = to;
+            }
+            for (int i = k - 1; i > 0; --i)
+                if (len[i] < (long long)floor_b) { len[i - 1] -= (long long)floor_b - len[i]; len[i] = (long long)floor_b; }
+        }
+        p.n = k;
+        for (int i = 0; i < k; ++i) p.cut[i + 1] = p.cut[i] + (size_t)len[i];
+        return p;
+    }
+    size_t len[OverlapPlan::kMaxChunks];
+    int n = 0;
+    size_t rest = n_blocks;
+    size_t l = std::max(floor_b, (size_t)(t.overlap_tail_frac * (double)n_blocks + 0.5));
+    if (rest < l + floor_b) l = rest;
+    for (;;) {
+        if (n == OverlapPlan::kMaxChunks - 1) l = rest;
+        len[n++] = l;
+        rest -= l;
+        if (rest == 0) break;
+        const size_t next = (size_t)((double)l / ratio);
+        l = rest <= next ? rest : (rest - next < floor_b ? rest - floor_b : next);
+    }
+    p.n = n;
+    for (int i = 0; i < n; ++i) p.cut[i + 1] = p.cut[i] + len[n - 1 - i];
+    return p;
+}
+
 const Tuning &tuning()
 {
 #ifdef OHS_EXPERIMENTS
@@ -102,6 +156,7 @@
     if (key == "force_overlap") return one(&t.force_overlap);
     if (key == "xcd_split") { if (!one(&t.xcd_split)) return false; if (t.xcd_split < 0 || t.xcd_split > 7) t.xcd_split = 0; return true; }
     if (key == "overlap_cuts") {
+        if (value.empty() || value == "rule") { t.overlap_cuts = Tuning().overlap_cuts; t.overlap_cuts_forced = 0; return true; }
         std::vector<double> c = {0.0};
         const char *p = value.c_str();
         while (*p && c.size() < 16) {
@@ -114,8 +169,11 @@
         c.push_back(1.0);
         if (c.size() < 3) return false;
         t.overlap_cuts = c;
-        return true;
-    }
+        t.overlap_cuts_forced = 1;
+        return true;
+    }
+    if (key == "overlap_ratio") { t.overlap_ratio = atof(value.c_str()); return t.overlap_ratio > 0.0; }
+    if (key == "overlap_tail_frac") { t.overlap_tail_frac = atof(value.c_str()); return t.overlap_tail_frac > 0.0 && t.overlap_tail_frac < 1.0; }
     if (key == "conv_cu_mask") {
         std::vector<unsigned> m;
         const char *p = value.c_str();
diff --git a/open_headstage_amd/csrc/tuning.h b/open_headstage_amd/csrc/tuning.h
--- a/open_headstage_amd/csrc/tuning.h
+++ b/open_headstage_amd/csrc/tuning.h
@@ -1,6 +1,7 @@
 #pragma once
 #include "experiments.h"
 
+#include <cstddef>
 #include <string>
 #include <vector>
 
@@ -24,6 +25,10 @@
     int eq_lds = 0;
     int no_overlap = 0, force_overlap = 0;
     int xcd_split = 0;
+    double overlap_tail_frac = 0.025;
+    double overlap_ratio = 0.16;
+    int overlap_min_blocks = 16;
+    int overlap_cuts_forced = 0;
     std::vector<double> overlap_cuts = {0.0, 0.25, 0.5, 0.75, 0.92, 0.98, 1.0};
     std::vector<unsigned> conv_cu_mask;
     int mac_no_xcd = 0;
@@ -44,6 +49,13 @@
     unsigned rt_poll_sleep = 0;
 };
 
+struct OverlapPlan {
+    static constexpr int kMaxChunks = 16;
+    int n = 1;
+    size_t cut[kMaxChunks + 1] = {};
+};
+OverlapPlan overlap_plan(size_t n_blocks, bool wave_ring, const Tuning &t);
+
 const Tuning &tuning();
 Tuning &tuning_rt();
 inline int rt_max_resident_load() { return __atomic_load_n(&tuning().rt_max_resident, __ATOMIC_RELAXED); }
```
